# OATML-Markslab/ProteinGym

Measured on AMD Instinct MI355X. Metric: mutants scored/sec (ESM-1v 650M masked-marginal), higher is better.
Workload: dtype f16x3 (fp32 operands split into 2 fp16 planes, 3 fp16 MFMAs per product, fp32 accumulate)

## Files before the change

### proteingym_amd/csrc/api_esm.hip

```cpp
#include "model.h"

namespace pgmi {

int create_esm(pgmi_model* m, const pgmi_config* cfg, const float* w, int64_t n_weights) {
    const size_t D = cfg->embed_dim, F = cfg->ffn_dim, V = cfg->vocab, dh = m->dh, Da = m->Da;
    BlobCursor c(m, w, n_weights);
    c.upload(&m->embed_tokens, V * D);
    if (cfg->arch == PGMI_ARCH_ESM1B) c.upload(&m->embed_positions, (size_t)(cfg->max_positions + 2) * D);
    if (cfg->emb_layer_norm_before) {
        c.upload(&m->lnb_w, D);
        c.upload(&m->lnb_b, D);
    }
    auto slot = [&](size_t col) -> size_t { return rotate_half_slot(col, dh); };
    const float qscale = 1.0f / sqrtf((float)dh);
    m->layers.resize(cfg->layers);
    std::vector<float> wq(3 * Da * D, 0.0f), bq(3 * Da, 0.0f), wo_r(D * Da, 0.0f);
    for (int l = 0; l < cfg->layers; ++l) {
        Layer& L = m->layers[l];
        c.upload(&L.ln1_w, D);
        c.upload(&L.ln1_b, D);
        pack_qkv_slots(c.take(3 * (D * D + D)), D, Da, slot, qscale, wq.data(), bq.data());
        c.linear(&L.wqkv, &L.wqkv16, wq.data(), wq.size(), D);
        c.upload(&L.bqkv, bq.data(), bq.size());
        pack_out_cols(c.take(D * D), D, Da, slot, wo_r.data());
        c.linear(&L.wo, &L.wo16, wo_r.data(), wo_r.size(), Da);
        c.upload(&L.bo, D);
        c.upload(&L.ln2_w, D);
        c.upload(&L.ln2_b, D);
        c.linear(&L.w1, &L.w116, F * D, D);
        c.upload(&L.b1, F);
        c.linear(&L.w2, &L.w216, D * F, F);
        c.upload(&L.b2, D);
    }
    c.upload(&m->lna_w, D);
    c.upload(&m->lna_b, D);
    c.linear(&m->hd_w, &m->hd16, D * D, D);
    c.upload(&m->hd_b, D);
    c.upload(&m->hln_w, D);
    c.upload(&m->hln_b, D);
    c.upload(&m->head_b, V);
    m->head_w = m->embed_tokens;
    return c.finish();
}

int ensure_rotary(pgmi_model* m, int T) {
    if ((!esm2_rotary(m->cfg.arch) && m->cfg.arch != PGMI_ARCH_ESMC) || T <= m->rot_len) return PGMI_OK;
    return upload_rotate_half(m, std::max(T, 1026));
}

int upload_rotate_half(pgmi_model* m, int n) {
    const int rh = m->rot_halves;
    float inv[64];
    const int half = m->dh / 2;
    for (int i = 0; i < half; ++i) inv[i] = 1.0f / powf(10000.0f, (float)(2 * i) / (float)m->dh);
    return upload_rotary(m, n, rh, [&](int t, int g, int i) {
        const int j = (rh == 1) ? i : 32 * g + i;
        return j < half ? (float)t * inv[j] : 0.0f;
    });
}

int run_encoder(pgmi_model* m, int B, int T, const int32_t* keep, int n_keep, bool* compacted) {
    const pgmi_config& c = m->cfg;
    const int M = B * T, D = c.embed_dim, F = c.ffn_dim, N1 = m->fc1_cols, H = c.heads, Da = m->Da;
    hipStream_t s = m->stream;
    if (c.arch == PGMI_ARCH_ESM1B && T > c.max_positions) {
        set_error("Sequence length %d above maximum sequence length of %d", T, c.max_positions);
        return PGMI_EINVAL;
    }
    int rc = ensure_rotary(m, T);
    if (!rc) rc = reset_pad_keys(m, B, T);
    if (rc) return rc;
    {
        ProfScope p(m, PGMI_K_EMBED, 0, (double)M * D * 4);
        launch_seq_stats(m->tokens, B, T, m->embed_gather ? 0 : c.token_dropout, m->denom, m->pos_idx, m->kv_len, s, m->mask_id);
        if (m->embed_gather) launch_gather_rows(m->embed_tokens, m->tokens, M, D, m->x, s);
        else launch_embed(m->tokens, m->denom, m->pos_idx, m->embed_tokens, m->embed_positions, c.token_dropout, M, T, D, m->x, s, m->mask_id);
        if (m->lnb_w) {
            launch_layernorm(m->x, m->lnb_w, m->lnb_b, M, D, 1e-5f, m->x, s);
            launch_zero_pad_rows(m->tokens, M, D, m->x, s);
        }
    }
    const double ln_bytes = 2.0 * M * D * 4;
    const int prec = c.precision;
    const int mode16 = (prec == PGMI_PREC_F16X3) ? 1 : 2;
    for (int l = 0; l < c.layers; ++l) {
        const Layer& L = m->layers[l];
        { ProfScope p(m, PGMI_K_LAYERNORM, 0, ln_bytes);
          if (prec == PGMI_PREC_FP32) launch_layernorm(m->x, L.ln1_w, L.ln1_b, M, D, 1e-5f, m->h, s);
          else launch_layernorm16(m->x, L.ln1_w, L.ln1_b, M, D, 1e-5f, m->h16, m->h16_plane, mode16, s); }
        const bool fused_qkv = prec != PGMI_PREC_FP32 && !L.q_ln;
        { ProfScope p(m, PGMI_K_GEMM_QKV, 2.0 * M * 3 * D * D, 0);
          if (fused_qkv)
              rc = launch_gemm16_qkv(m->h16, m->h16_plane, L.wqkv16.p, L.wqkv16.plane, L.bqkv, M, Da, D, L.wqkv16.out_scale,
                                     m->qk16, m->qk16_plane, m->vt16, m->vt16_plane, m->rot_cos, m->rot_sin,
                                     esm2_rotary(c.arch), T, m->Hs, m->gemm_variant, s, m->rot_halves, prec == PGMI_PREC_BF16);
          else
              rc = linear(m, m->h, m->h16, m->h16_plane, L.wqkv, L.wqkv16, L.bqkv, nullptr, m->qkv, nullptr, 0, M, 3 * Da, D, EPI_NONE);
          if (rc) return rc; }
        { ProfScope p(m, PGMI_K_ATTENTION, 4.0 * M * T * D, L.q_ln ? (double)M * D * 20 : 0);
          if (L.q_ln && (rc = launch_qkln_prep(m->qkv, L.q_ln, L.k_ln, 1e-5f, m->rot_cos, m->rot_sin, B, T, H, m->qk16, m->qk16_plane,
                                               m->vt16, m->vt16_plane, s)))
              return rc;
          const bool v2 = prec != PGMI_PREC_FP32;
          if (esm2_rotary(c.arch) && !v2) launch_rotary(m->qkv, m->rot_cos, m->rot_sin, M, T, m->Hs, s, m->rot_halves);
          if (v2) {
              AttLaunch a;
              a.qk16 = m->qk16, a.qk_plane = m->qk16_plane, a.vt16 = m->vt16, a.vt_plane = m->vt16_plane;
              a.B = B, a.T = T, a.H = H, a.head_dim = m->rot_halves * kHeadDim;
              a.kv_len = m->kv_len;
              a.out = prec == PGMI_PREC_F16X3 ? ATT_OUT_SPLIT : ATT_OUT_BF16;
              a.ctx16 = m->h16;
              a.stream = s;
              rc = launch_attention_f16x3_v2(a);
          } else {
              rc = launch_attention_f32(m->qkv, m->kv_len, B, T, H, m->h, s, m->rot_halves * kHeadDim);
          }
          if (rc) return rc; }
        if (keep && m->keep_rows && l == c.layers - 1) {
            const int R = n_keep;
            ProfScope p(m, PGMI_K_KEPT_ROWS, 2.0 * R * D * (Da + N1 + F), 0);
            launch_gather_rows(m->x, keep, R, D, m->qkv, s);
            if (prec == PGMI_PREC_FP32) launch_gather_rows(m->h, keep, R, Da, m->g, s);
            else
                launch_gather_rows(reinterpret_cast<const float*>(m->h16), keep, R, prec == PGMI_PREC_F16X3 ? Da : Da / 2,
                                   reinterpret_cast<float*>(m->g16), s);
            rc = linear(m, m->g, m->g16, m->g16_plane, L.wo, L.wo16, L.bo, m->qkv, m->x, nullptr, 0, R, D, Da, EPI_NONE);
            if (rc) return rc;
            if (prec == PGMI_PREC_FP32) launch_layernorm(m->x, L.ln2_w, L.ln2_b, R, D, 1e-5f, m->h, s);
            else launch_layernorm16(m->x, L.ln2_w, L.ln2_b, R, D, 1e-5f, m->h16, m->h16_plane, mode16, s);
            rc = linear(m, m->h, m->h16, m->h16_plane, L.w1, L.w116, L.b1, nullptr,
                        prec == PGMI_PREC_FP32 ? m->g : nullptr, prec == PGMI_PREC_FP32 ? nullptr : m->g16, m->g16_plane,
                        R, N1, D, m->fc1_epi);
            if (rc) return rc;
            rc = linear(m, m->g, m->g16, m->g16_plane, L.w2, L.w216, L.b2, m->x, m->x, nullptr, 0, R, D, F, EPI_NONE);
            if (rc) return rc;
            if (compacted) *compacted = true;
            break;
        }
        { ProfScope p(m, PGMI_K_GEMM_OUT, 2.0 * M * D * D, 0);
          rc = linear(m, m->h, m->h16, m->h16_plane, L.wo, L.wo16, L.bo, m->x, m->x, nullptr, 0, M, D, Da, EPI_NONE);
          if (rc) return rc; }
        { ProfScope p(m, PGMI_K_LAYERNORM, 0, ln_bytes);
          if (prec == PGMI_PREC_FP32) launch_layernorm(m->x, L.ln2_w, L.ln2_b, M, D, 1e-5f, m->h, s);
          else launch_layernorm16(m->x, L.ln2_w, L.ln2_b, M, D, 1e-5f, m->h16, m->h16_plane, mode16, s); }
        { ProfScope p(m, PGMI_K_GEMM_FC1, 2.0 * M * N1 * D, 0);
          rc = linear(m, m->h, m->h16, m->h16_plane, L.w1, L.w116, L.b1, nullptr,
                      prec == PGMI_PREC_FP32 ? m->g : nullptr, prec == PGMI_PREC_FP32 ? nullptr : m->g16, m->g16_plane,
                      M, N1, D, m->fc1_epi);
          if (rc) return rc; }
        { ProfScope p(m, PGMI_K_GEMM_FC2, 2.0 * M * F * D, 0);
          rc = linear(m, m->g, m->g16, m->g16_plane, L.w2, L.w216, L.b2, m->x, m->x, nullptr, 0, M, D, F, EPI_NONE);
          if (rc) return rc; }
    }
    PGMI_HIP(hipGetLastError());
    return PGMI_OK;
}

int run_head(pgmi_model* m, int R, const int32_t* row_idx) {
    const pgmi_config& c = m->cfg;
    ProfScope p(m, PGMI_K_HEAD, 2.0 * R * c.embed_dim * (c.embed_dim + c.vocab), 0);
    int rc = head_hidden(m, R, row_idx);
    if (rc) return rc;
    launch_vocab_logsoftmax(m->g, m->head_w, m->head_b, R, c.embed_dim, c.vocab, m->lp, m->nonfinite, m->stream);
    PGMI_HIP(hipGetLastError());
    return PGMI_OK;
}

int head_hidden(pgmi_model* m, int R, const int32_t* row_idx) {
    const pgmi_config& c = m->cfg;
    const int D = c.embed_dim;
    hipStream_t s = m->stream;
    const int prec = c.precision;
    const float* src = m->x;
    if (row_idx) {
        launch_gather_rows(m->x, row_idx, R, D, m->h, s);
        src = m->h;
    }
    if (prec == PGMI_PREC_FP32) launch_layernorm(src, m->lna_w, m->lna_b, R, D, 1e-5f, m->h, s);
    else launch_layernorm16(src, m->lna_w, m->lna_b, R, D, 1e-5f, m->h16, m->h16_plane, prec == PGMI_PREC_F16X3 ? 1 : 2, s);
    int rc = linear(m, m->h, m->h16, m->h16_plane, m->hd_w, m->hd16, m->hd_b, nullptr, m->g, nullptr, 0, R, D, D, EPI_GELU);
    if (rc) return rc;
    launch_layernorm(m->g, m->hln_w, m->hln_b, R, D, 1e-5f, m->g, s);
    return PGMI_OK;
}


int run_rows(pgmi_model* m, int B, int T, int R, const int32_t* row_idx) {
    bool compacted = false;
    int rc = run_encoder(m, B, T, row_idx, R, &compacted);
    if (rc) return rc;
    return run_head(m, R, compacted ? nullptr : row_idx);
}

}

extern "C" {

int pgmi_token_logprobs(pgmi_model* m, const int32_t* tokens, int B, int T, float* out) {
    if (!m || !tokens || !out || B <= 0 || T <= 0) { set_error("bad argument"); return PGMI_EINVAL; }
    if (m->cfg.arch == PGMI_ARCH_SAPROT) { set_error("SaProt models are scored with pgmi_saprot_token_logprobs / pgmi_saprot_group_logprobs"); return PGMI_EINVAL; }
    if (T + 31 > m->max_rows) { set_error("T=%d exceeds workspace rows %d", T, m->max_rows); return PGMI_EINVAL; }
    int rc = check_tokens(tokens, B, T);
    if (rc) return rc;
    PGMI_HIP(hipSetDevice(m->device));
    const int V = m->cfg.vocab;
    rc = for_each_chunk(m, B, T, [&](int b0, int bc) {
        PGMI_HIP(hipMemcpyAsync(m->tokens, tokens + (size_t)b0 * T, (size_t)bc * T * 4, hipMemcpyHostToDevice, m->stream));
        int rc = run_rows(m, bc, T, bc * T, nullptr);
        if (rc) return rc;
        PGMI_HIP(hipMemcpyAsync(out + (size_t)b0 * T * V, m->lp, (size_t)bc * T * V * 4, hipMemcpyDeviceToHost, m->stream));
        return PGMI_OK;
    });
    return rc ? rc : check_nonfinite(m);
}

int pgmi_masked_logprobs(pgmi_model* m, const int32_t* tokens, const int32_t* mask_pos, int B, int T, float* out) {
    if (!m || !tokens || !mask_pos || !out || B <= 0 || T <= 0) { set_error("bad argument"); return PGMI_EINVAL; }
    if (m->cfg.arch == PGMI_ARCH_SAPROT) { set_error("SaProt models are scored with pgmi_saprot_token_logprobs / pgmi_saprot_group_logprobs"); return PGMI_EINVAL; }
    if (m->cfg.arch == PGMI_ARCH_ESMC && T + 31 > m->max_rows) { set_error("T=%d exceeds workspace rows %d", T, m->max_rows); return PGMI_EINVAL; }
    if (T > m->max_rows) { set_error("T=%d exceeds workspace rows %d", T, m->max_rows); return PGMI_EINVAL; }
    int rc = check_tokens(tokens, B, T);
    if (rc) return rc;
    for (int b = 0; b < B; ++b)
        if (mask_pos[b] < 0 || mask_pos[b] >= T) { set_error("mask_pos[%d]=%d out of range", b, mask_pos[b]); return PGMI_EINVAL; }
    PGMI_HIP(hipSetDevice(m->device));
    const int V = m->cfg.vocab;
    std::vector<int32_t> ridx;
    rc = for_each_chunk(m, B, T, [&](int b0, int bc) {
        ridx.resize(bc);
        for (int b = 0; b < bc; ++b) ridx[b] = b * T + mask_pos[b0 + b];
        PGMI_HIP(hipMemcpyAsync(m->tokens, tokens + (size_t)b0 * T, (size_t)bc * T * 4, hipMemcpyHostToDevice, m->stream));
        PGMI_HIP(hipMemcpyAsync(m->aux_i, mask_pos + b0, (size_t)bc * 4, hipMemcpyHostToDevice, m->stream));
        PGMI_HIP(hipMemcpyAsync(m->row_idx, ridx.data(), (size_t)bc * 4, hipMemcpyHostToDevice, m->stream));
        launch_apply_mask(m->tokens, m->aux_i, bc, T, m->stream);
        int rc = run_rows(m, bc, T, bc, m->row_idx);
        if (rc) return rc;
        PGMI_HIP(hipMemcpyAsync(out + (size_t)b0 * V, m->lp, (size_t)bc * V * 4, hipMemcpyDeviceToHost, m->stream));
        return PGMI_OK;
    });
    return rc ? rc : check_nonfinite(m);
}

int pgmi_assay_create(pgmi_model* m, const int32_t* wt_tokens, int n_tok, const int32_t* positions, int P,
                      int window, const int32_t* sub_pos, const int32_t* sub_wt, const int32_t* sub_mt,
                      const int64_t* mut_off, int64_t n_mut, pgmi_assay** out) {
    if (!out) { set_error("null out"); return PGMI_EINVAL; }
    *out = nullptr;
    if (!m || !wt_tokens || n_tok <= 0 || P < 0 || (P > 0 && !positions) || window <= 0 || n_mut < 0) { set_error("bad argument"); return PGMI_EINVAL; }
    if (m->cfg.arch == PGMI_ARCH_ESMC) { set_error("ESM C assays run through pgmi_masked_logprobs (their window rule is not pgmi_optimal_window)"); return PGMI_EINVAL; }
    if (m->cfg.arch == PGMI_ARCH_SAPROT) { set_error("SaProt assays run through pgmi_saprot_group_logprobs (position sets, no window)"); return PGMI_EINVAL; }
    for (int i = 0; i < n_tok; ++i)
        if (wt_tokens[i] < 0 || wt_tokens[i] >= PGMI_VOCAB || wt_tokens[i] == PGMI_TOK_PAD) { set_error("wt token %d invalid at %d", wt_tokens[i], i); return PGMI_EINVAL; }
    const int T = std::min(n_tok, window);
    if (T > m->max_rows) { set_error("T=%d exceeds workspace rows %d", T, m->max_rows); return PGMI_EINVAL; }
    std::vector<int32_t> ws(P), mr(P);
    for (int i = 0; i < P; ++i) {
        if (positions[i] < 0 || positions[i] >= n_tok) { set_error("position %d out of range", positions[i]); return PGMI_EINVAL; }
        int s, e;
        pgmi_optimal_window(positions[i], n_tok, window, &s, &e);
        if (e - s != T) { set_error("internal: window length %d != %d", e - s, T); return PGMI_EINVAL; }
        ws[i] = s;
        mr[i] = positions[i] - s;
    }
    const int64_t n_sub = n_mut ? mut_off[n_mut] : 0;
    for (int64_t k = 0; k < n_sub; ++k)
        if (sub_pos[k] < 0 || sub_pos[k] >= n_tok || sub_wt[k] < 0 || sub_wt[k] >= PGMI_VOCAB || sub_mt[k] < 0 || sub_mt[k] >= PGMI_VOCAB) {
            set_error("substitution %lld out of range", (long long)k);
            return PGMI_EINVAL;
        }
    PGMI_HIP(hipSetDevice(m->device));
    pgmi_assay* a = new pgmi_assay();
    a->m = m; a->n_tok = n_tok; a->P = P; a->T = T; a->n_mut = n_mut; a->n_sub = n_sub;
    int rc = dev_upload(a->allocs, &a->wt, wt_tokens, (size_t)n_tok);
    if (!rc) rc = dev_upload(a->allocs, &a->positions, positions, (size_t)P);
    if (!rc) rc = dev_upload(a->allocs, &a->win_start, ws.data(), (size_t)P);
    if (!rc) rc = dev_upload(a->allocs, &a->mask_rel, mr.data(), (size_t)P);
    if (!rc) rc = dev_upload(a->allocs, &a->sub_pos, sub_pos, (size_t)n_sub);
    if (!rc) rc = dev_upload(a->allocs, &a->sub_wt, sub_wt, (size_t)n_sub);
    if (!rc) rc = dev_upload(a->allocs, &a->sub_mt, sub_mt, (size_t)n_sub);
    if (!rc) rc = dev_upload(a->allocs, &a->mut_off, mut_off, (size_t)(n_mut + 1));
    if (!rc) rc = dev_alloc(a->allocs, &a->table, (size_t)n_tok * PGMI_VOCAB);
    if (!rc) rc = dev_alloc(a->allocs, &a->scores, (size_t)n_mut);
    if (rc) { pgmi_assay_destroy(a); return rc; }
    m->assays.push_back(a);
    *out = a;
    return PGMI_OK;
}

void pgmi_assay_destroy(pgmi_assay* a) {
    if (!a) return;
    if (a->m) {
        hipSetDevice(a->m->device);
        hipStreamSynchronize(a->m->stream);
        auto& v = a->m->assays;
        v.erase(std::remove(v.begin(), v.end(), a), v.end());
    }
    for (void* p : a->allocs) hipFree(p);
    delete a;
}

int pgmi_assay_run(pgmi_model* m, pgmi_assay* a, double* scores_host, float* table_host, double* scores_dev) {
    if (!m || !a || a->m != m) { set_error("bad model/assay handle (assay belongs to another or a destroyed model)"); return PGMI_EINVAL; }
    PGMI_HIP(hipSetDevice(m->device));
    hipStream_t s = m->stream;
    const int T = a->T, V = m->cfg.vocab;
    const int per = rows_per_chunk(m, T);
    launch_fill_f32(a->table, (int64_t)a->n_tok * V, NAN, s);
    for (int p0 = 0; p0 < a->P; p0 += per) {
        const int bc = std::min(per, a->P - p0);
        launch_make_masked_windows(a->wt, a->win_start + p0, a->mask_rel + p0, bc, T, m->tokens, s);
        launch_row_index(a->mask_rel + p0, bc, T, m->row_idx, s);
        int rc = run_rows(m, bc, T, bc, m->row_idx);
        if (rc) return rc;
        launch_scatter_rows(m->lp, a->positions + p0, bc, V, a->table, s);
    }
    {
        ProfScope p(m, PGMI_K_SCORE, 0, (double)a->n_sub * 20);
        launch_score_mutants(a->table, V, a->sub_pos, a->sub_wt, a->sub_mt, a->mut_off, a->n_mut, a->scores, s);
    }
    PGMI_HIP(hipGetLastError());
    if (scores_dev && a->n_mut) PGMI_HIP(hipMemcpyAsync(scores_dev, a->scores, (size_t)a->n_mut * 8, hipMemcpyDeviceToDevice, s));
    if (scores_host && a->n_mut) PGMI_HIP(hipMemcpyAsync(scores_host, a->scores, (size_t)a->n_mut * 8, hipMemcpyDeviceToHost, s));
    if (table_host) PGMI_HIP(hipMemcpyAsync(table_host, a->table, (size_t)a->n_tok * V * 4, hipMemcpyDeviceToHost, s));
    PGMI_HIP(hipStreamSynchronize(s));
    return check_nonfinite(m);
}

int pgmi_pppl_create(pgmi_model* m, const uint8_t* tokens, const int64_t* seq_off, int64_t n_seq, pgmi_pppl** out) {
    if (!out) { set_error("null out"); return PGMI_EINVAL; }
    *out = nullptr;
    if (!m || !tokens || !seq_off || n_seq <= 0 || n_seq > 0x7fffffff) { set_error("bad argument"); return PGMI_EINVAL; }
    if (m->cfg.arch != PGMI_ARCH_ESM1B && m->cfg.arch != PGMI_ARCH_ESM2) { set_error("pseudo-ppl needs an ESM-1b/1v/ESM2 model"); return PGMI_EINVAL; }
    if (seq_off[0] != 0) { set_error("seq_off[0] must be 0"); return PGMI_EINVAL; }
    for (int64_t n = 0; n < n_seq; ++n) {
        const int64_t len = seq_off[n + 1] - seq_off[n];
        if (len < 2 || len > (1 << 24)) { set_error("sequence %lld has %lld tokens", (long long)n, (long long)len); return PGMI_EINVAL; }
        const uint8_t* t = tokens + seq_off[n];
        for (int64_t i = 0; i < len; ++i)
            if (t[i] >= PGMI_VOCAB || t[i] == PGMI_TOK_PAD) { set_error("token id %d invalid at sequence %lld, position %lld", (int)t[i], (long long)n, (long long)i); return PGMI_EINVAL; }
    }
    PGMI_HIP(hipSetDevice(m->device));
    pgmi_pppl* q = new pgmi_pppl();
    q->m = m;
    q->N = n_seq;
    q->off.assign(seq_off, seq_off + n_seq + 1);
    int rc = dev_upload(q->allocs, &q->tok8, tokens, (size_t)seq_off[n_seq]);
    if (!rc) rc = dev_upload(q->allocs, &q->off_dev, seq_off, (size_t)n_seq + 1);
    if (rc) { for (void* p : q->allocs) hipFree(p); delete q; return rc; }
    m->pppls.push_back(q);
    *out = q;
    return PGMI_OK;
}

void pgmi_pppl_destroy(pgmi_pppl* q) {
    if (!q) return;
    if (q->m) {
        hipSetDevice(q->m->device);
        hipStreamSynchronize(q->m->stream);
        auto& v = q->m->pppls;
        v.erase(std::remove(v.begin(), v.end(), q), v.end());
    }
    for (void* p : q->allocs) hipFree(p);
    delete q;
}

int64_t pgmi_pppl_rows(const pgmi_pppl* q, int64_t first, int64_t count) {
    if (!q || first < 0 || count < 0 || first + count > q->N) return -1;
    int64_t r = 0;
    for (int64_t n = first; n < first + count; ++n) r += std::max<int64_t>(0, q->off[n + 1] - q->off[n] - 4);
    return r;
}

int pgmi_pppl_run(pgmi_model* m, pgmi_pppl* q, int64_t first, int64_t count, double* scores_host, float* terms_host,
                  double* scores_dev) {
    if (!m || !q || q->m != m) { set_error("bad model/library handle (library belongs to another or a destroyed model)"); return PGMI_EINVAL; }
    if (first < 0 || count <= 0 || first + count > q->N) { set_error("sequence range [%lld, %lld) outside the library of %lld", (long long)first, (long long)(first + count), (long long)q->N); return PGMI_EINVAL; }
    PGMI_HIP(hipSetDevice(m->device));
    hipStream_t s = m->stream;
    const int J = (int)count, V = m->cfg.vocab;
    std::vector<int32_t> sid(J);
    for (int j = 0; j < J; ++j) sid[j] = (int32_t)(first + j);
    auto len_of = [&](int32_t n) { return q->off[n + 1] - q->off[n]; };
    std::stable_sort(sid.begin(), sid.end(), [&](int32_t a, int32_t b) { return len_of(a) > len_of(b); });
    std::vector<int64_t> rp((size_t)J + 1);
    rp[0] = 0;
    for (int j = 0; j < J; ++j) rp[j + 1] = rp[j] + std::max<int64_t>(0, len_of(sid[j]) - 4);
    const int64_t R = rp[J];
    const int64_t Tmax = len_of(sid[0]);
    if (R > 0 && Tmax + 31 > m->max_rows) { set_error("T=%lld exceeds workspace rows %d", (long long)Tmax, m->max_rows); return PGMI_EINVAL; }
    if (R > 0 && m->cfg.arch == PGMI_ARCH_ESM1B && Tmax > m->cfg.max_positions) {
        set_error("Sequence length %lld above maximum sequence length of %d", (long long)Tmax, m->cfg.max_positions);
        return PGMI_EINVAL;
    }
    std::vector<void*> pool;
    auto cleanup = [&]() { for (void* p : pool) hipFree(p); };
    int32_t* d_sid = nullptr;
    int64_t* d_rp = nullptr;
    float* d_terms = nullptr;
    double* d_out = nullptr;
    int rc = dev_upload(pool, &d_sid, sid.data(), (size_t)J);
    if (!rc) rc = dev_upload(pool, &d_rp, rp.data(), (size_t)J + 1);
    if (!rc) rc = dev_alloc(pool, &d_terms, (size_t)R);
    if (!rc) rc = dev_alloc(pool, &d_out, (size_t)J);
    if (rc) { cleanup(); return rc; }
    q->last_rows = R; q->last_chunks = 0; q->last_tokens = 0; q->last_padded = 0;
    int j0 = 0;
    for (int64_t g0 = 0; g0 < R;) {
        while (rp[j0 + 1] <= g0) ++j0;
        const int T = (int)len_of(sid[j0]);
        const int bc = (int)std::min<int64_t>(rows_per_chunk(m, T), R - g0);
        launch_make_pppl_rows(q->tok8, q->off_dev, d_sid, d_rp, J, g0, bc, T, m->tokens, m->row_idx, m->aux_i, s);
        rc = run_rows(m, bc, T, bc, m->row_idx);
        if (rc) { hipStreamSynchronize(s); cleanup(); return rc; }
        launch_pppl_pick(m->lp, m->aux_i, bc, V, d_terms + g0, s);
        q->last_chunks += 1;
        q->last_padded += (int64_t)bc * T;
        g0 += bc;
        if ((q->last_chunks & 63) == 0 && g0 < R && (rc = check_nonfinite(m)) != PGMI_OK) { cleanup(); return rc; }
    }
    for (int j = 0; j < J; ++j) q->last_tokens += (rp[j + 1] - rp[j]) * len_of(sid[j]);
    {
        ProfScope p(m, PGMI_K_SCORE, 0, (double)R * 4);
        launch_pppl_sum(d_terms, d_rp, d_sid, J, first, d_out, s);
    }
    hipError_t e = hipGetLastError();
    if (e == hipSuccess && scores_dev) e = hipMemcpyAsync(scores_dev, d_out, (size_t)J * 8, hipMemcpyDeviceToDevice, s);
    if (e == hipSuccess && scores_host) e = hipMemcpyAsync(scores_host, d_out, (size_t)J * 8, hipMemcpyDeviceToHost, s);
    std::vector<float> sorted_terms;
    if (e == hipSuccess && terms_host && R > 0) {
        sorted_terms.resize((size_t)R);
        e = hipMemcpyAsync(sorted_terms.data(), d_terms, (size_t)R * 4, hipMemcpyDeviceToHost, s);
    }
    if (e == hipSuccess) e = hipStreamSynchronize(s);
    cleanup();
    if (e != hipSuccess) { set_error("pseudo-ppl run failed: %s", hipGetErrorString(e)); return PGMI_EHIP; }
    if (terms_host && R > 0) {
        std::vector<int64_t> dst((size_t)J + 1, 0);
        for (int k = 0; k < J; ++k) dst[k + 1] = dst[k] + std::max<int64_t>(0, len_of((int32_t)(first + k)) - 4);
        for (int j = 0; j < J; ++j)
            std::copy(sorted_terms.begin() + rp[j], sorted_terms.begin() + rp[j + 1], terms_host + dst[sid[j] - first]);
    }
    return check_nonfinite(m);
}

int pgmi_pppl_stats(const pgmi_pppl* q, int64_t* rows, int64_t* chunks, int64_t* tokens, int64_t* padded_tokens) {
    if (!q) { set_error("null library"); return PGMI_EINVAL; }
    if (rows) *rows = q->last_rows;
    if (chunks) *chunks = q->last_chunks;
    if (tokens) *tokens = q->last_tokens;
    if (padded_tokens) *padded_tokens = q->last_padded;
    return PGMI_OK;
}

}
```

### proteingym_amd/csrc/api_model.hip

```cpp
#include "model.h"

namespace pgmi {

static thread_local char g_err[1024] = "";
void set_error(const char* fmt, ...) {
    va_list ap;
    va_start(ap, fmt);
    vsnprintf(g_err, sizeof(g_err), fmt, ap);
    va_end(ap);
}

int prof_drain(pgmi_model* m) {
    if (m->events_used == 0) return PGMI_OK;
    PGMI_HIP(hipStreamSynchronize(m->stream));
    for (size_t i = 0; i < m->events_used; ++i) {
        float ms = 0.f;
        PGMI_HIP(hipEventElapsedTime(&ms, m->events[i].start, m->events[i].stop));
        m->prof_ms[m->events[i].cls] += ms;
    }
    m->events_used = 0;
    return PGMI_OK;
}

int check_cfg(const pgmi_config* c) {
    if (!c) { set_error("null config"); return PGMI_EINVAL; }
    if (c->abi_version != PGMI_ABI_VERSION) { set_error("ABI version mismatch: got %d, library is %d", c->abi_version, PGMI_ABI_VERSION); return PGMI_EINVAL; }
    if (c->arch != PGMI_ARCH_ESM1B && c->arch != PGMI_ARCH_ESM2 && c->arch != PGMI_ARCH_TRANCEPTION && c->arch != PGMI_ARCH_MSA &&
        c->arch != PGMI_ARCH_PROGEN2 && c->arch != PGMI_ARCH_GPT && c->arch != PGMI_ARCH_ESMC && c->arch != PGMI_ARCH_SAPROT) { set_error("unknown arch %d", c->arch); return PGMI_EINVAL; }
    if (c->layers <= 0 || c->embed_dim <= 0 || c->heads <= 0 || c->ffn_dim <= 0) { set_error("non-positive model dimension"); return PGMI_EINVAL; }
    if (c->arch == PGMI_ARCH_ESMC) {
        if (c->precision != PGMI_PREC_F16X3) { set_error("ESM C is available in precision f16x3 only"); return PGMI_EINVAL; }
        if (c->embed_dim % 32 || c->embed_dim != c->heads * kHeadDim) { set_error("ESM C needs head_dim 64 and d %% 32 == 0 (embed_dim %d, heads %d)", c->embed_dim, c->heads); return PGMI_EINVAL; }
        if (c->embed_dim > 2048) { set_error("ESM C: embed_dim %d above the 2048 this build supports", c->embed_dim); return PGMI_EINVAL; }
        if (c->ffn_dim % 32) { set_error("ESM C: the SwiGLU hidden width %d must be a multiple of 32", c->ffn_dim); return PGMI_EINVAL; }
        if (c->vocab != PGMI_ESMC_VOCAB) { set_error("ESM C vocab must be %d", PGMI_ESMC_VOCAB); return PGMI_EINVAL; }
        return PGMI_OK;
    }
    {
        const int dh = c->embed_dim / c->heads;
        const bool pg2 = c->arch == PGMI_ARCH_PROGEN2;
        const bool esm_layout = c->arch == PGMI_ARCH_ESM1B || c->arch == PGMI_ARCH_ESM2 || c->arch == PGMI_ARCH_GPT || c->arch == PGMI_ARCH_SAPROT;
        const bool ok = c->embed_dim % c->heads == 0 &&
                        (dh == kHeadDim || (dh < kHeadDim && dh % 2 == 0 && esm_layout) || (dh == 2 * kHeadDim && esm_layout) ||
                         (pg2 && dh % 2 == 0 && dh <= 4 * kHeadDim));
        if (pg2 && !ok && c->embed_dim % c->heads == 0 && dh > 4 * kHeadDim) {
            set_error("unsupported head_dim %d (embed_dim %d / heads %d): ProGen2 runs even head dims up to 256", dh, c->embed_dim, c->heads);
            return PGMI_EINVAL;
        }
        if (!ok) { set_error("unsupported head_dim %d (embed_dim %d / heads %d): this build supports head_dim 64, even head dims below 64 and head_dim 128 (ESM)", dh, c->embed_dim, c->heads); return PGMI_EINVAL; }
    }
    if (c->embed_dim % 32 || c->ffn_dim % 32) { set_error("embed_dim and ffn_dim must be multiples of 32"); return PGMI_EINVAL; }
    if (c->arch == PGMI_ARCH_TRANCEPTION) {
        if (c->vocab != 25) { set_error("Tranception vocab must be 25"); return PGMI_EINVAL; }
        if (c->heads % 4) { set_error("Invalid number of heads. Tranception requires the number of heads to be a multiple of 4."); return PGMI_EINVAL; }
        if (c->precision != PGMI_PREC_F16X3) { set_error("Tranception is available in precision f16x3 only"); return PGMI_EINVAL; }
        if (c->max_positions <= 0) { set_error("Tranception needs max_positions = n_ctx"); return PGMI_EINVAL; }
    } else if (c->arch == PGMI_ARCH_PROGEN2) {
        if (c->vocab != PGMI_PG2_VOCAB) { set_error("ProGen2 vocab must be %d", PGMI_PG2_VOCAB); return PGMI_EINVAL; }
        if (c->heads % 8) { set_error("ProGen2 needs the number of heads to be a multiple of 8 (mp_num = 8), got %d", c->heads); return PGMI_EINVAL; }
        if (c->precision != PGMI_PREC_F16X3) { set_error("ProGen2 is available in precision f16x3 only"); return PGMI_EINVAL; }
        if (c->max_positions <= 0) { set_error("ProGen2 needs max_positions = n_positions"); return PGMI_EINVAL; }
    } else if (c->arch == PGMI_ARCH_GPT) {
        if (c->vocab < 2) { set_error("causal decoder vocab must be at least 2, got %d", c->vocab); return PGMI_EINVAL; }
        if (c->precision != PGMI_PREC_F16X3) { set_error("the causal decoder (RITA / ProtGPT2) is available in precision f16x3 only"); return PGMI_EINVAL; }
        if (c->max_positions <= 0) { set_error("the causal decoder needs max_positions = n_positions / max_seq_len"); return PGMI_EINVAL; }
    } else if (c->arch == PGMI_ARCH_SAPROT) {
        if (c->vocab != PGMI_SAPROT_VOCAB) { set_error("SaProt vocab must be %d (5 specials + 21 x 21 residue tokens)", PGMI_SAPROT_VOCAB); return PGMI_EINVAL; }
        if (c->max_positions != 0) { set_error("SaProt has rotary positions: max_positions must be 0"); return PGMI_EINVAL; }
    } else if (c->vocab != PGMI_VOCAB) { set_error("vocab must be %d", PGMI_VOCAB); return PGMI_EINVAL; }
    if (c->arch == PGMI_ARCH_ESM1B && c->max_positions <= 0) { set_error("ESM-1b arch needs max_positions"); return PGMI_EINVAL; }
    if (c->arch == PGMI_ARCH_MSA) {
        if (c->max_positions <= 0) { set_error("MSA Transformer needs max_positions"); return PGMI_EINVAL; }
        if (c->embed_dim != c->heads * kHeadDim) { set_error("MSA Transformer: head_dim must be 64"); return PGMI_EINVAL; }
        if (c->precision != PGMI_PREC_F16X3) { set_error("MSA Transformer is available in precision f16x3 only"); return PGMI_EINVAL; }
    }
    if (c->precision != PGMI_PREC_FP32 && c->precision != PGMI_PREC_F16X3 && c->precision != PGMI_PREC_BF16) { set_error("unknown precision %d", c->precision); return PGMI_EINVAL; }
    if (c->precision == PGMI_PREC_BF16 && (c->embed_dim % 64 || c->ffn_dim % 64)) { set_error("precision bf16 needs embed_dim and ffn_dim to be multiples of 64"); return PGMI_EINVAL; }
    return PGMI_OK;
}

int check_tokens(const int32_t* tokens, int B, int T, int n_ids) {
    for (int b = 0; b < B; ++b) {
        const int32_t* t = tokens + (size_t)b * T;
        bool seen_pad = false;
        if (t[0] == PGMI_TOK_PAD) { set_error("sequence %d is empty (all <pad>)", b); return PGMI_EINVAL; }
        for (int i = 0; i < T; ++i) {
            if (t[i] < 0 || t[i] >= n_ids) { set_error("token id %d out of range at [%d,%d]", t[i], b, i); return PGMI_EINVAL; }
            if (t[i] == PGMI_TOK_PAD) seen_pad = true;
            else if (seen_pad) { set_error("interior <pad> at [%d,%d]: only trailing padding is supported", b, i); return PGMI_EINVAL; }
        }
    }
    return PGMI_OK;
}

int check_vocab(const int32_t* tokens, int B, int T, int V) {
    for (int b = 0; b < B; ++b)
        for (int t = 0; t < T; ++t) {
            const int tk = tokens[(size_t)b * T + t];
            if (tk < 0 || tk >= V) { set_error("token id %d out of range at [%d,%d]", tk, b, t); return PGMI_EINVAL; }
        }
    return PGMI_OK;
}

int env_int(const char* name, int dflt) {
    const char* v = getenv(name);
    return v ? atoi(v) : dflt;
}

int make_w16(std::vector<void*>& pool, const float* host, size_t n, size_t K, int precision, hipStream_t s, W16* out) {
    float mx = 0.f;
    for (size_t i = 0; i < n; ++i) mx = std::max(mx, fabsf(host[i]));
    float scale = 1.0f;
    const int planes = (precision == PGMI_PREC_F16X3) ? 2 : 1;
    if (precision == PGMI_PREC_F16X3 && mx > 0.f && std::isfinite(mx)) scale = exp2f(floorf(log2f(16384.0f / mx)));
    float* tmp = nullptr;
    hipError_t e = hipMalloc(reinterpret_cast<void**>(&tmp), n * sizeof(float));
    if (e != hipSuccess) { set_error("hipMalloc failed: %s", hipGetErrorString(e)); return PGMI_ENOMEM; }
    int rc = dev_alloc(pool, &out->p, n * planes);
    if (rc) { hipFree(tmp); return rc; }
    e = hipMemcpy(tmp, host, n * sizeof(float), hipMemcpyHostToDevice);
    if (e == hipSuccess) {
        launch_split16(tmp, (int64_t)n, scale, precision == PGMI_PREC_BF16 ? 1 : 0, (int)K, out->p, s);
        e = hipStreamSynchronize(s);
    }
    hipFree(tmp);
    if (e != hipSuccess) { set_error("weight split failed: %s", hipGetErrorString(e)); return PGMI_EHIP; }
    out->plane = n;
    out->out_scale = 1.0f / scale;
    return PGMI_OK;
}

int linear(pgmi_model* m, const float* in32, const unsigned short* in16, size_t in_plane, const float* W32,
           const W16& w16, const float* bias, const float* residual, float* out32, unsigned short* out16,
           size_t out_plane, int M, int N, int K, int epi) {
    if (m->cfg.precision == PGMI_PREC_FP32)
        return launch_gemm_f32(in32, W32, bias, residual, out32, M, N, K, epi, m->stream);
    const bool bf = m->cfg.precision == PGMI_PREC_BF16;
    return launch_gemm16(in16, in_plane, w16.p, w16.plane, bias, residual, out32, out16, out_plane, M, N, K, epi,
                         w16.out_scale, bf ? 1 : 2, bf, m->gemm_variant, m->stream);
}

int check_nonfinite(pgmi_model* m) {
    if (m->cfg.precision == PGMI_PREC_FP32) return PGMI_OK;
    int32_t flag = 0;
    PGMI_HIP(hipMemcpyAsync(&flag, m->nonfinite, 4, hipMemcpyDeviceToHost, m->stream));
    PGMI_HIP(hipStreamSynchronize(m->stream));
    if (flag) {
        PGMI_HIP(hipMemsetAsync(m->nonfinite, 0, 4, m->stream));
        set_error("non-finite log-probabilities: an activation left the fp16/bf16 range in precision mode %d; "
                  "re-run with precision fp32", m->cfg.precision);
        return PGMI_EOVERFLOW;
    }
    return PGMI_OK;
}

int reset_pad_keys(pgmi_model* m, int B, int T) {
    if (!m->vt16 || (B == m->last_B && T == m->last_T)) return PGMI_OK;
    PGMI_HIP(hipMemsetAsync(m->vt16, 0, m->vt16_plane * 2 * sizeof(unsigned short), m->stream));
    m->last_B = B;
    m->last_T = T;
    return PGMI_OK;
}

}

extern "C" {

int pgmi_abi_version(void) { return PGMI_ABI_VERSION; }

const char* pgmi_last_error(void) { return g_err; }

int pgmi_device_count(void) {
    int n = 0;
    if (hipGetDeviceCount(&n) != hipSuccess) return 0;
    return n;
}

int64_t pgmi_weight_count(const pgmi_config* c) {
    if (!c || c->layers <= 0 || c->embed_dim <= 0 || c->ffn_dim <= 0) return -1;
    const int64_t D = c->embed_dim, F = c->ffn_dim, V = c->vocab;
    if (c->arch == PGMI_ARCH_TRANCEPTION) {
        const int64_t conv = 3 * ((64 * 3 + 64) + (64 * 5 + 64) + (64 * 7 + 64));
        return V * D + (int64_t)c->layers * (2 * D + (D * 3 * D + 3 * D) + conv + (D * D + D) + 2 * D + (D * F + F) + (F * D + D)) + 2 * D + V * D;
    }
    if (c->arch == PGMI_ARCH_PROGEN2)
        return V * D + (int64_t)c->layers * (2 * D + 3 * D * D + D * D + (F * D + F) + (D * F + D)) + 2 * D + V * D + V;
    if (c->arch == PGMI_ARCH_GPT) return -1;
    if (c->arch == PGMI_ARCH_ESMC) return esmc_weight_count(c);
    if (c->arch == PGMI_ARCH_MSA) {
        const int64_t attn = 2 * D + 4 * (D * D + D);
        return V * D + (int64_t)(c->max_positions + 2) * D + 1024 * D + 2 * D +
               (int64_t)c->layers * (2 * attn + 2 * D + (F * D + F) + (D * F + D)) + 2 * D + (D * D + D) + 2 * D + V;
    }
    int64_t n = V * D;
    if (c->arch == PGMI_ARCH_ESM1B) n += (int64_t)(c->max_positions + 2) * D;
    if (c->emb_layer_norm_before) n += 2 * D;
    n += (int64_t)c->layers * (2 * D + 4 * (D * D + D) + 2 * D + (F * D + F) + (D * F + D));
    n += 2 * D + (D * D + D) + 2 * D + V;
    return n;
}

int pgmi_model_create(const pgmi_config* cfg, const float* w, int64_t n_weights, int device, pgmi_model** out) {
    if (cfg && cfg->arch == PGMI_ARCH_PROGEN2) {
        if (out) *out = nullptr;
        set_error("ProGen2 models are created with pgmi_pg2_model_create (it takes rotary_dim)");
        return PGMI_EINVAL;
    }
    if (cfg && cfg->arch == PGMI_ARCH_GPT) {
        if (out) *out = nullptr;
        set_error("causal decoder models are created with pgmi_gpt_model_create (it takes pos_kind)");
        return PGMI_EINVAL;
    }
    if (cfg && cfg->arch == PGMI_ARCH_SAPROT) {
        if (out) *out = nullptr;
        set_error("SaProt models are created with pgmi_saprot_model_create (it takes the tokenizer's <mask> id)");
        return PGMI_EINVAL;
    }
    return model_create(cfg, w, n_weights, device, out, 0);
}

}

namespace pgmi {

static int alloc_workspace(pgmi_model* m) {
    const pgmi_config& c = m->cfg;
    const size_t R = m->max_rows, D = c.embed_dim, F = c.ffn_dim, V = c.vocab, Da = m->Da;
    const size_t Dw = std::max(D, Da);
    const bool f32mode = c.precision == PGMI_PREC_FP32;
    int rc = PGMI_OK;
    auto alloc = [&](auto** p, size_t n) { if (!rc) rc = dev_alloc(m->allocs, p, n); };
    alloc(&m->x, R * D);
    alloc(&m->h, R * Dw);
    alloc(&m->qkv, R * 3 * Da);
    alloc(&m->g, R * (f32mode ? std::max(F, D) : D));
    if (!f32mode) {
        const size_t planes = c.precision == PGMI_PREC_F16X3 ? 2 : 1;
        m->h16_plane = R * Dw;
        m->g16_plane = R * F;
        alloc(&m->h16, m->h16_plane * planes);
        alloc(&m->g16, m->g16_plane * planes);
    }
    alloc(&m->nonfinite, (size_t)1);
    if (!f32mode) {
        m->qk16_plane = R * 2 * Da;
        m->vt16_plane = R * Da;
        alloc(&m->qk16, m->qk16_plane * 2);
        alloc(&m->vt16, m->vt16_plane * 2);
    }
    if (c.arch == PGMI_ARCH_MSA) {
        alloc(&m->xt, R * D);
        alloc(&m->msa_kv_len, (size_t)2048);
    }
    alloc(&m->lp, (c.arch == PGMI_ARCH_GPT && V > kWave ? (size_t)m->gpt_head_rows : R) * V);
    alloc(&m->denom, R);
    alloc(&m->tokens, R);
    alloc(&m->pos_idx, R);
    alloc(&m->kv_len, R);
    alloc(&m->row_idx, R);
    alloc(&m->aux_i, R);
    if (rc) return rc;
    PGMI_HIP(hipMemset(m->nonfinite, 0, 4));
    if (m->vt16) PGMI_HIP(hipMemset(m->vt16, 0, m->vt16_plane * 2 * sizeof(unsigned short)));
    return PGMI_OK;
}

int model_create(const pgmi_config* cfg, const float* w, int64_t n_weights, int device, pgmi_model** out, int arch_arg) {
    if (!out) { set_error("null out"); return PGMI_EINVAL; }
    *out = nullptr;
    int rc = check_cfg(cfg);
    if (rc) return rc;
    const int64_t need = cfg->arch == PGMI_ARCH_GPT ? gpt_weight_count(cfg, arch_arg) : pgmi_weight_count(cfg);
    if (need < 0) { set_error("causal decoder pos_kind %d: must be PGMI_GPT_POS_ROTARY or PGMI_GPT_POS_LEARNED", arch_arg); return PGMI_EINVAL; }
    if (!w || n_weights != need) {
        set_error("weight blob has %lld elements, config needs %lld", (long long)n_weights, (long long)need);
        return PGMI_EINVAL;
    }
    const int ndev = pgmi_device_count();
    if (ndev <= 0) { set_error("no HIP device visible (libpgmi has no CPU fallback)"); return PGMI_ENODEV; }
    if (device < 0 || device >= ndev) { set_error("device %d out of range (%d visible)", device, ndev); return PGMI_EINVAL; }
    PGMI_HIP(hipSetDevice(device));
    pgmi_model* m = new pgmi_model();
    m->cfg = *cfg;
    m->device = device;
    if (hipStreamCreateWithFlags(&m->stream, hipStreamNonBlocking) != hipSuccess) { set_error("hipStreamCreate failed"); delete m; return PGMI_EHIP; }
    m->dh = cfg->embed_dim / cfg->heads;
    m->rot_halves = m->dh > 2 * kHeadDim ? 4 : m->dh > kHeadDim ? 2 : 1;
    m->Hs = cfg->heads * m->rot_halves;
    m->Da = m->Hs * kHeadDim;
    m->ln_eps = cfg->ln_eps > 0.f ? cfg->ln_eps : 1e-5f;
    m->max_rows = std::max(cfg->max_rows > 0 ? cfg->max_rows : 98304, 2048);
    const size_t V = cfg->vocab;
    const std::vector<float> zeros(std::max({3 * (size_t)m->Da, (V + 63) / 64 * 64, (size_t)cfg->embed_dim, V, (size_t)cfg->heads}), 0.0f);
    rc = dev_upload(m->allocs, &m->zeros, zeros.data(), zeros.size());
    m->fc1_cols = cfg->ffn_dim;
    if (!rc) switch (cfg->arch) {
        case PGMI_ARCH_TRANCEPTION: rc = create_tranception(m, cfg, w, n_weights); break;
        case PGMI_ARCH_MSA: rc = create_msa(m, cfg, w, n_weights); break;
        case PGMI_ARCH_PROGEN2: rc = create_progen2(m, cfg, w, n_weights, arch_arg); break;
        case PGMI_ARCH_GPT: rc = create_gpt(m, cfg, w, n_weights, arch_arg); break;
        case PGMI_ARCH_ESMC: rc = create_esmc(m, cfg, w, n_weights); break;
        case PGMI_ARCH_SAPROT: rc = create_saprot(m, cfg, w, n_weights, arch_arg); break;
        default: rc = create_esm(m, cfg, w, n_weights);
    }
    if (!rc) rc = alloc_workspace(m);
    if (rc) { pgmi_model_destroy(m); return rc; }
    m->keep_rows = env_int("PGMI_KEEP_ROWS", 1);
    gemm_options_from_env();
    m->gemm_variant = env_int("PGMI_GEMM_VARIANT", 0);
    *out = m;
    return PGMI_OK;
}

}

extern "C" {

void pgmi_model_destroy(pgmi_model* m) {
    if (!m) return;
    hipSetDevice(m->device);
    if (m->stream) hipStreamSynchronize(m->stream);
    for (pgmi_assay* a : m->assays) {
        for (void* p : a->allocs) hipFree(p);
        a->allocs.clear();
        a->m = nullptr;
    }
    m->assays.clear();
    for (pgmi_pppl* q : m->pppls) {
        for (void* p : q->allocs) hipFree(p);
        q->allocs.clear();
        q->m = nullptr;
    }
    m->pppls.clear();
    for (auto& e : m->events) { hipEventDestroy(e.start); hipEventDestroy(e.stop); }
    for (void* p : m->allocs) hipFree(p);
    if (m->stream) hipStreamDestroy(m->stream);
    delete m;
}

int pgmi_model_device(const pgmi_model* m) { return m ? m->device : -1; }

int pgmi_set_option(const char* name, int64_t value) {
    if (!name) { set_error("null option name"); return PGMI_EINVAL; }
    int rc = gemm_set_option(name, (long long)value);
    if (rc) rc = att_set_option(name, (long long)value);
    if (rc) rc = eve_set_option(name, (long long)value);
    if (rc) set_error("unknown option '%s' (gemm_half_tail, gemm_max_rows, att_xcd_local, att_v3, eve_max_rows, eve_fixed_sample)", name);
    return rc;
}

int pgmi_synchronize(pgmi_model* m) {
    if (!m) { set_error("null model"); return PGMI_EINVAL; }
    PGMI_HIP(hipStreamSynchronize(m->stream));
    return PGMI_OK;
}

int pgmi_profile_enable(pgmi_model* m, int on) {
    if (!m) { set_error("null model"); return PGMI_EINVAL; }
    int rc = prof_drain(m);
    m->prof = on != 0;
    return rc;
}

int pgmi_profile_reset(pgmi_model* m) {
    if (!m) { set_error("null model"); return PGMI_EINVAL; }
    int rc = prof_drain(m);
    for (int i = 0; i < PGMI_K_COUNT; ++i) { m->prof_ms[i] = 0; m->prof_n[i] = 0; m->prof_flops[i] = 0; m->prof_bytes[i] = 0; }
    return rc;
}

int pgmi_profile_get(pgmi_model* m, int k, double* ms, int64_t* launches, double* flops, double* bytes) {
    if (!m || k < 0 || k >= PGMI_K_COUNT) { set_error("bad argument"); return PGMI_EINVAL; }
    int rc = prof_drain(m);
    if (rc) return rc;
    if (ms) *ms = m->prof_ms[k];
    if (launches) *launches = m->prof_n[k];
    if (flops) *flops = m->prof_flops[k];
    if (bytes) *bytes = m->prof_bytes[k];
    return PGMI_OK;
}

}
```

### proteingym_amd/csrc/attention_f16.hip

```cpp
#include <stdlib.h>
#include <string.h>
#include <algorithm>

#include "attention_f16_common.h"

namespace pgmi {

template <int WPB, int OUT, int NSTG, int DH = 64, bool RAG = false, int DO = DH>
__global__ __launch_bounds__(WPB * 64) void attention_f16x3_v2_kernel(
    const unsigned short* __restrict__ qk16, size_t qk_plane, const unsigned short* __restrict__ vt16,
    size_t vt_plane, const int32_t* __restrict__ kv_len, const float* __restrict__ slopes, int T, int H,
    int Tp, float* __restrict__ ctx, unsigned short* __restrict__ ctx16, RagMap rag, int dense_nblk, int nseq) {
    constexpr float defer_thr = kAttDefer;
    constexpr int NT = WPB * 64;
    constexpr int KCPR = DH / 8;
    constexpr int KCH = AKT * KCPR, VCH = DO * 4;
    constexpr int NSL = DH / DO;
    static_assert(NSL == 1 || (OUT == ATT_OUT_SPLIT && !RAG), "sliced context: split-plane output of dense launches only");
    constexpr int STG_CH = 2 * KCH + 2 * VCH;
    constexpr int NWI = STG_CH / 64;
    static_assert(NWI % WPB == 0, "the wave-instructions of a stage divide evenly over the waves");
    constexpr int NDMA = NWI / WPB;
    constexpr int NS = DH / 16, ND = DO / 32;
    extern __shared__ __attribute__((aligned(16))) u32x4 lds[];

    int b, h, qblk_dense, hs;
    if (RAG) {
        b = rag.ent_seq[blockIdx.x];
        hs = blockIdx.y;
        qblk_dense = 0;
    } else if (dense_nblk > 0) {
        const int pair = xcd_local_pair(dense_nblk, qblk_dense);
        if (pair >= nseq * H * NSL) return;
        b = pair / (H * NSL);
        hs = pair - b * (H * NSL);
    } else {
        b = blockIdx.z;
        hs = blockIdx.y;
        qblk_dense = blockIdx.x;
    }
    h = hs / NSL;
    const int d0 = (hs - h * NSL) * DO;
    const int tid = threadIdx.x, lane = tid & 63;
    const int wave = __builtin_amdgcn_readfirstlane(tid >> 6);
    const int r = lane & 31, kh = lane >> 5;
    const int D = H * DH;
    const int Tk = (!RAG && kv_len) ? kv_len[b] : T;
    const int p0 = RAG ? rag.seq_p[b] : 0, a0 = p0 & ~(AKT - 1), kt0 = a0 / AKT;
    const int qblk = RAG ? rag.ent_j[blockIdx.x] : qblk_dense;
    const int row0 = RAG ? rag.seq_q[b] : b * T, rrow0 = RAG ? rag.seq_q[rag.seq_root[b]] : 0;
    const int orow0 = RAG ? rag.seq_off[b] - p0 : b * T;
    const int Tpo = RAG ? (T - a0 + 31) / 32 * 32 : Tp;
    const int q0 = a0 + (qblk * WPB + wave) * 32;
    const bool active = q0 < T;

    constexpr bool q_lds = NSTG >= 3;
    u32x4 qh[NS], ql[NS];
    if (!q_lds) {
        const int qrow = min(q0 + r, T - 1);
        const unsigned short* qp = qk16 + ((size_t)row0 + (qrow - a0)) * (2 * D) + h * DH + kh * 8;
#pragma unroll
        for (int s = 0; s < NS; ++s) {
            qh[s] = *reinterpret_cast<const u32x4*>(qp + s * 16);
            ql[s] = *reinterpret_cast<const u32x4*>(qp + qk_plane + s * 16);
        }
    }

    const size_t seq_halfs = (size_t)T * (2 * D), vt_halfs = (size_t)DH * Tp;
    const unsigned long long qk_bytes = std::min<unsigned long long>(0xFFFFFFFFull, (unsigned long long)qk_plane * 2ull + seq_halfs * 2ull);
    const unsigned long long vt_bytes = std::min<unsigned long long>(0xFFFFFFFFull, (unsigned long long)vt_plane * 2ull + vt_halfs * 2ull);
    const __amdgpu_buffer_rsrc_t rsQK = operand_rsrc(qk16 + (size_t)row0 * (2 * D), qk_bytes);
    const __amdgpu_buffer_rsrc_t rsVT = operand_rsrc(vt16 + (RAG ? (size_t)rag.seq_vt[b] + (size_t)h * DH * Tpo : ((size_t)b * H + h) * vt_halfs), vt_bytes);
    const __amdgpu_buffer_rsrc_t rsQKr = operand_rsrc(qk16 + (size_t)rrow0 * (2 * D), qk_bytes);
    const __amdgpu_buffer_rsrc_t rsVTr = operand_rsrc(vt16 + (RAG ? (size_t)rag.seq_vt[rag.seq_root[b]] + (size_t)h * DH * Tp : (size_t)0), vt_bytes);
    const bool causal = slopes != nullptr;
    const int last_q = min(T, a0 + (qblk * WPB + WPB) * 32);
    const int nkt = causal ? (min(Tk, last_q) + AKT - 1) / AKT : (Tk + AKT - 1) / AKT;
    int voff[NDMA], voff_last[NDMA], voff_root[NDMA], sbase[NDMA], sstep[NDMA], slot0[NDMA];
    bool is_k[NDMA];
#pragma unroll
    for (int i = 0; i < NDMA; ++i) {
        int wi = wave + WPB * i;
        if (wi >= NWI) wi -= NWI;
        slot0[i] = wi * 64;
        is_k[i] = wi < 2 * KCH / 64;
        if (is_k[i]) {
            const int p = wi / (KCH / 64), key = ((wi % (KCH / 64)) * 64 + lane) / KCPR;
            const int c = (lane % KCPR) ^ k_swizzle<DH>(key);
            voff[i] = voff_root[i] = key * (2 * D) * 2 + c * 16;
            voff_last[i] = min(key, T - 1 - (nkt - 1) * AKT) * (2 * D) * 2 + c * 16;
            sbase[i] = (int)((unsigned int)p * (unsigned int)qk_plane * 2u + (unsigned int)(D + h * DH) * 2u);
            sstep[i] = AKT * (2 * D) * 2;
        } else {
            const int wv = wi - 2 * KCH / 64, p = wv / (VCH / 64), g = (wv % (VCH / 64)) * 64 + lane;
            const int d = g >> 2, c = (g & 3) ^ ((d >> 2) & 3);
            voff[i] = voff_last[i] = (d0 + d) * Tpo * 2 + c * 16;
            voff_root[i] = (d0 + d) * Tp * 2 + c * 16;
            sbase[i] = (int)((unsigned int)p * (unsigned int)vt_plane * 2u);
            sstep[i] = (AKT / 8) * 16;
        }
    }
    auto issue_tile = [&](int kt, int buf) {
        u32x4* base = lds + buf * STG_CH;
        const bool from_root = RAG && kt < kt0;
#pragma unroll
        for (int i = 0; i < NDMA; ++i) {
            const int vo = from_root ? voff_root[i] : ((kt == nkt - 1) ? voff_last[i] : voff[i]);
            const int so = sbase[i] + (from_root ? kt : kt - kt0) * sstep[i];
            if (is_k[i]) __builtin_amdgcn_raw_ptr_buffer_load_lds(from_root ? rsQKr : rsQK, (__attribute__((address_space(3))) void*)(base + slot0[i]), 16, vo, so, 0, 0);
            else __builtin_amdgcn_raw_ptr_buffer_load_lds(from_root ? rsVTr : rsVT, (__attribute__((address_space(3))) void*)(base + slot0[i]), 16, vo, so, 0, 0);
        }
    };

    constexpr float kLog2e = 1.4426950408889634f;
    const float slope2 = causal ? slopes[h] * kLog2e : 0.0f;
    if (q_lds) {
        issue_tile(0, 0);
        u32x4* qbase = lds + STG_CH + wave * (2 * KCH);
        if (active) {
            constexpr int NQ = 2 * KCH / 64;
#pragma unroll
            for (int i = 0; i < NQ; ++i) {
                const int f = i * 64 + lane, pq = f / KCH, row = (f % KCH) / KCPR;
                const int c = (f % KCPR) ^ k_swizzle<DH>(row);
                const int vo = (int)(((unsigned int)(min(q0 + row, T - 1) - a0) * (unsigned int)(2 * D) + (unsigned int)(h * DH)) * 2u + (unsigned int)c * 16u);
                const int so = (int)((unsigned int)pq * (unsigned int)qk_plane * 2u);
                __builtin_amdgcn_raw_ptr_buffer_load_lds(rsQK, (__attribute__((address_space(3))) void*)(qbase + i * 64), 16, vo, so, 0, 0);
            }
        }
        asm volatile("s_waitcnt vmcnt(0)" ::: "memory");
        if (active) {
#pragma unroll
            for (int s = 0; s < NS; ++s) {
                const int ci = r * KCPR + ((2 * s + kh) ^ k_swizzle<DH>(r));
                qh[s] = qbase[ci];
                ql[s] = qbase[KCH + ci];
            }
        }
        asm volatile("s_waitcnt lgkmcnt(0)" ::: "memory");
        __builtin_amdgcn_s_barrier();
        asm volatile("" ::: "memory");
#pragma unroll
        for (int t = 1; t < NSTG - 1; ++t)
            if (t < nkt) issue_tile(t, t);
    } else {
#pragma unroll
        for (int t = 0; t < NSTG - 1; ++t)
            if (t < nkt) issue_tile(t, t);
    }

    f32x16 om[ND], oc[ND];
#pragma unroll
    for (int dt = 0; dt < ND; ++dt)
#pragma unroll
        for (int v = 0; v < 16; ++v) { om[dt][v] = 0.f; oc[dt][v] = 0.f; }
    float m_run = -INFINITY, l_run = 0.f;
    constexpr float kInvLo = 1.0f / kLoScale;

    const f32x16 zero16 = {0.f, 0.f, 0.f, 0.f, 0.f, 0.f, 0.f, 0.f, 0.f, 0.f, 0.f, 0.f, 0.f, 0.f, 0.f, 0.f};
    auto wanted = [&](int kt) -> bool { return active && !(causal && kt * AKT > q0 + 31); };
    auto scores = [&](int buf, f32x16& sm, f32x16& sc) {
        const u32x4* Kb = lds + buf * STG_CH;
#pragma unroll
        for (int s = 0; s < NS; ++s) {
            const int ci = r * KCPR + ((2 * s + kh) ^ k_swizzle<DH>(r));
            const u32x4 kfh = Kb[ci], kfl = Kb[KCH + ci];
            sc = mfma_h(kfh, ql[s], s == 0 ? zero16 : sc);
            sc = mfma_h(kfl, qh[s], sc);
            sm = mfma_h(kfh, qh[s], s == 0 ? zero16 : sm);
        }
    };
    auto wait_tile = [&](int younger) {
        if (younger >= 2) asm volatile("s_waitcnt vmcnt(%0)" ::"n"(2 * NDMA) : "memory");
        else if (younger == 1) asm volatile("s_waitcnt vmcnt(%0)" ::"n"(NDMA) : "memory");
        else asm volatile("s_waitcnt vmcnt(0)" ::: "memory");
    };
    int cur = 0;
    for (int kt = 0; kt < nkt; ++kt) {
        wait_tile(min(NSTG - 2, nkt - 1 - kt));
        __builtin_amdgcn_s_barrier();
        asm volatile("" ::: "memory");
        if (kt + NSTG - 1 < nkt) issue_tile(kt + NSTG - 1, (cur == 0) ? NSTG - 1 : cur - 1);
        if (wanted(kt)) {
            const u32x4* Vb = lds + cur * STG_CH + 2 * KCH;
            f32x16 sm, sc;
            scores(cur, sm, sc);
            float st[16];
            if (causal) {
                const float kb = (float)(kt * AKT + 4 * kh);
#pragma unroll
                for (int v = 0; v < 16; ++v)
                    st[v] = fmaf(slope2, kb + (float)((v & 3) + 8 * (v >> 2)), fmaf(sc[v], kInvLo, sm[v]));
                if (kt * AKT + AKT - 1 > q0) {
#pragma unroll
                    for (int v = 0; v < 16; ++v) {
                        const int key = kt * AKT + (v & 3) + 8 * (v >> 2) + 4 * kh;
                        if (key > q0 + r) st[v] = -INFINITY;
                    }
                }
            } else {
#pragma unroll
                for (int v = 0; v < 16; ++v) st[v] = fmaf(sc[v], kInvLo, sm[v]);
            }
            if (kt * AKT + AKT > Tk) {
#pragma unroll
                for (int v = 0; v < 16; ++v) {
                    const int key = kt * AKT + (v & 3) + 8 * (v >> 2) + 4 * kh;
                    if (key >= Tk) st[v] = -INFINITY;
                }
            }
            float mloc = st[0];
#pragma unroll
            for (int v = 1; v < 16; ++v) mloc = fmaxf(mloc, st[v]);
            {
                const unsigned int mu = __builtin_bit_cast(unsigned int, mloc);
                const auto sw = __builtin_amdgcn_permlane32_swap(mu, mu, false, false);
                const unsigned int s0 = sw[0], s1 = sw[1];
                mloc = fmaxf(__builtin_bit_cast(float, s0), __builtin_bit_cast(float, s1));
            }
            const float m_new = fmaxf(m_run, mloc);
            if (!__all(m_new <= m_run + defer_thr)) {
                const bool moved = m_new > m_run + defer_thr;
                const float alpha = moved ? __builtin_amdgcn_exp2f(m_run - m_new) : 1.0f;
                l_run *= alpha;
#pragma unroll
                for (int dt = 0; dt < ND; ++dt)
#pragma unroll
                    for (int v = 0; v < 16; ++v) { om[dt][v] *= alpha; oc[dt][v] *= alpha; }
                if (moved) m_run = m_new;
            }
            const float mb = m_run - 10.0f;
            typedef float f32x2 __attribute__((ext_vector_type(2)));
#pragma unroll
            for (int v = 0; v < 16; v += 2) {
                const f32x2 dlt = f32x2{st[v], st[v + 1]} - f32x2{mb, mb};
                st[v] = __builtin_amdgcn_exp2f(dlt[0]);
                st[v + 1] = __builtin_amdgcn_exp2f(dlt[1]);
            }
            l_run += ((st[0] + st[1]) + (st[2] + st[3])) + ((st[4] + st[5]) + (st[6] + st[7])) +
                     (((st[8] + st[9]) + (st[10] + st[11])) + ((st[12] + st[13]) + (st[14] + st[15])));
#pragma unroll
            for (int m = 0; m < 2; ++m) {
                u32x4 ph, pl;
#pragma unroll
                for (int e = 0; e < 4; ++e) {
                    const u32x2 p = split_p(st[8 * m + 2 * e], st[8 * m + 2 * e + 1]);
                    ph[e] = p[0];
                    pl[e] = p[1];
                }
#pragma unroll
                for (int dt = 0; dt < ND; ++dt) {
                    const int ci = v_chunk(dt * 32 + r, m, kh);
                    const u32x4 vfh = Vb[ci], vfl = Vb[VCH + ci];
                    oc[dt] = mfma_h(vfh, pl, oc[dt]);
                    oc[dt] = mfma_h(vfl, ph, oc[dt]);
                    om[dt] = mfma_h(vfh, ph, om[dt]);
                }
            }
        }
        cur = (cur == NSTG - 1) ? 0 : cur + 1;
    }

    if (active) {
        const float l_tot = l_run + __shfl_xor(l_run, 32);
        const float inv = 1.0f / l_tot;
        const bool row_ok = q0 + r < T && q0 + r >= p0;
        const size_t orow = (size_t)(orow0 + max(min(q0 + r, T - 1), p0));
        if (OUT == ATT_OUT_BF16) store_ctx_bf16<ND>(om, oc, inv, kInvLo, row_ok, ctx16 + orow * (size_t)D + (size_t)h * DH, kh);
        else if (OUT == ATT_OUT_SPLIT) store_ctx_split<ND>(om, oc, inv, kInvLo, row_ok, ctx16 + orow * (size_t)(2 * D) + (size_t)((h * DH + d0) / 32) * 64, kh);
        else if (row_ok) store_ctx_f32<ND>(om, oc, inv, kInvLo, ctx + (size_t)(orow0 + q0 + r) * D + (size_t)h * DH + 4 * kh);
    }
}


using Att16v2Kernel = decltype(&attention_f16x3_v2_kernel<4, ATT_OUT_F32, 3, 64, false, 64>);
struct Att16v2Inst { int wpb, out, head_dim; bool rag; Att16v2Kernel fn; size_t lds_bytes; };
template <int WPB, int OUT, int NSTG, int DH, bool RAG = false, int DO = DH>
static constexpr Att16v2Inst att16v2_inst() {
    return {WPB, OUT, DH, RAG, attention_f16x3_v2_kernel<WPB, OUT, NSTG, DH, RAG, DO>, (size_t)NSTG * (8 * DH + 8 * DO) * 16};
}
static const Att16v2Inst kAtt16v2[] = {
    att16v2_inst<1, ATT_OUT_F32, 3, 64>(),   att16v2_inst<2, ATT_OUT_F32, 3, 64>(),   att16v2_inst<4, ATT_OUT_F32, 3, 64>(),
    att16v2_inst<1, ATT_OUT_SPLIT, 3, 64>(), att16v2_inst<2, ATT_OUT_SPLIT, 3, 64>(), att16v2_inst<4, ATT_OUT_SPLIT, 3, 64>(),
    att16v2_inst<1, ATT_OUT_BF16, 3, 64>(),  att16v2_inst<2, ATT_OUT_BF16, 3, 64>(),  att16v2_inst<4, ATT_OUT_BF16, 3, 64>(),
    att16v2_inst<1, ATT_OUT_SPLIT, 3, 64, true>(), att16v2_inst<2, ATT_OUT_SPLIT, 3, 64, true>(), att16v2_inst<4, ATT_OUT_SPLIT, 3, 64, true>(),
    att16v2_inst<4, ATT_OUT_F32, 3, 128>(),  att16v2_inst<4, ATT_OUT_SPLIT, 3, 128>(), att16v2_inst<4, ATT_OUT_BF16, 3, 128>(),
    att16v2_inst<4, ATT_OUT_SPLIT, 2, 256, false, 128>(),
};

static int launch_att16v2(const AttLaunch& a, int wpb, dim3 grid, const RagMap* rag, int dense_nblk) {
    for (const Att16v2Inst& k : kAtt16v2) {
        if (k.wpb != wpb || k.out != a.out || k.head_dim != a.head_dim || k.rag != (rag != nullptr)) continue;
        if (k.lds_bytes > 65536) {
            hipError_t e = hipFuncSetAttribute(reinterpret_cast<const void*>(k.fn), hipFuncAttributeMaxDynamicSharedMemorySize, (int)k.lds_bytes);
            if (e != hipSuccess) { set_error("hipFuncSetAttribute: %s", hipGetErrorString(e)); return PGMI_EHIP; }
        }
        hipLaunchKernelGGL(k.fn, grid, dim3(wpb * 64), k.lds_bytes, a.stream, a.qk16, a.qk_plane, a.vt16, a.vt_plane, a.kv_len, a.slopes,
                           a.T, a.H, (a.T + 31) / 32 * 32, a.ctx, a.ctx16, rag ? *rag : RagMap{}, dense_nblk, a.B);
        PGMI_HIP(hipGetLastError());
        return PGMI_OK;
    }
    set_error("attention_f16x3_v2: no kernel for %d waves, output %d, head_dim %d%s", wpb, (int)a.out, a.head_dim, rag ? ", ragged" : "");
    return PGMI_EINVAL;
}

static int g_att_xcd_local = -1;
int att_set_option(const char* name, long long value) {
    if (!strcmp(name, "att_xcd_local")) { g_att_xcd_local = (int)value; return PGMI_OK; }
    if (!strcmp(name, "att_v3")) { att_v3_set_option((int)value); return PGMI_OK; }
    return PGMI_EINVAL;
}
static dim3 dense_grid(int nblk, int H, int B, int* dense_nblk) {
    if (g_att_xcd_local == 0 || (g_att_xcd_local < 0 && nblk < 2)) { *dense_nblk = 0; return dim3(nblk, H, B); }
    *dense_nblk = nblk;
    const long long pairs = (long long)H * B, groups = (pairs + 7) / 8;
    return dim3((unsigned)(groups * 8 * nblk), 1, 1);
}

int att16_waves_per_block(int T) {
    const int n32 = (T + 31) / 32, nblk = (n32 + 3) / 4;
    const int wpb = (n32 + nblk - 1) / nblk;
    return wpb == 3 ? 4 : wpb;
}

static int check_operand_range(const char* who, const AttLaunch& a) {
    const unsigned long long Tp = (unsigned long long)(a.T + 31) / 32 * 32;
    const unsigned long long seq_bytes = (unsigned long long)a.T * 2ull * (unsigned long long)a.H * (unsigned long long)a.head_dim * 2ull;
    const unsigned long long vt_bytes = (unsigned long long)a.head_dim * Tp * 2ull;
    if ((unsigned long long)a.qk_plane * 2ull + seq_bytes >= (1ull << 32) || (unsigned long long)a.vt_plane * 2ull + vt_bytes >= (1ull << 32)) {
        set_error("%s: operand planes of %zu / %zu halfs exceed the 32-bit offset range of the K / V^T DMA "
                  "(plane stride + one sequence must stay below 4 GiB: create the model with a smaller max_rows)", who, a.qk_plane, a.vt_plane);
        return PGMI_EINVAL;
    }
    return PGMI_OK;
}

int launch_attention_f16x3_v2(const AttLaunch& a) {
    const int B = a.B, T = a.T, H = a.H, head_dim = a.head_dim;
    if (B <= 0 || T <= 0 || H <= 0 || a.out < ATT_OUT_F32 || a.out > ATT_OUT_BF16 || (head_dim != 64 && head_dim != 128 && head_dim != 256)) {
        set_error("attention_f16x3_v2: bad arguments B=%d T=%d H=%d out=%d head_dim=%d", B, T, H, (int)a.out, head_dim);
        return PGMI_EINVAL;
    }
    const int n32 = (T + 31) / 32, Tp = n32 * 32;
    int rc = check_operand_range("attention_f16x3_v2", a);
    if (rc) return rc;
    int dn = 0;
    if (head_dim == 256) {
        if (a.qkv || a.conv || !a.slopes || a.out != ATT_OUT_SPLIT) { set_error("attention_f16x3_v2: head_dim 256 is the causal, fused-QKV, split-plane-output flavour only"); return PGMI_EINVAL; }
        const dim3 grid = dense_grid((n32 + 3) / 4, 2 * H, B, &dn);
        return launch_att16v2(a, 4, grid, nullptr, dn);
    }
    if (head_dim == 128) {
        if (a.qkv || a.conv) { set_error("attention_f16x3_v2: head_dim 128 needs operands from the fused QKV projection"); return PGMI_EINVAL; }
        const dim3 grid = dense_grid((n32 + 3) / 4, H, B, &dn);
        return launch_att16v2(a, 4, grid, nullptr, dn);
    }
    if (a.qkv && a.conv && a.rotary) { set_error("attention_f16x3_v2: depth-wise convolution and rotary together are not a model this library knows"); return PGMI_EINVAL; }
    if (a.qkv && a.conv && H % 4) { set_error("attention_f16x3_v2: the depth-wise convolution has four head groups, H = %d is not a multiple of 4", H); return PGMI_EINVAL; }
    if (a.qkv && a.conv)
        launch_qkv_prep_conv(dim3(n32, H, B), a.stream, a.qkv, a.conv, T, H, Tp, a.qk16, a.qk_plane, a.vt16, a.vt_plane, nullptr);
    else if (a.qkv)
        launch_qkv_prep(dim3(n32, H, B), a.stream, a.qkv, a.cos_t, a.sin_t, a.rotary, T, H, Tp, a.qk16, a.qk_plane, a.vt16, a.vt_plane);
    const int wpb = att16_waves_per_block(T);
    const dim3 grid = dense_grid((n32 + wpb - 1) / wpb, H, B, &dn);
    return att_v3_serves(a) ? launch_att16v3(a, wpb, grid, dn) : launch_att16v2(a, wpb, grid, nullptr, dn);
}

int launch_attention_tr_ragged(const AttLaunch& a, const AttRagged& rg) {
    const int T = a.T, H = a.H;
    if (T <= 0 || H <= 0 || !a.qkv || !a.conv || !a.slopes || a.head_dim != 64 || a.out != ATT_OUT_SPLIT || rg.n_tiles <= 0 || rg.n_blocks <= 0) {
        set_error("attention_tr_ragged: bad arguments T=%d H=%d tiles=%d blocks=%d", T, H, rg.n_tiles, rg.n_blocks);
        return PGMI_EINVAL;
    }
    const int rc = check_operand_range("attention_tr_ragged", a);
    if (rc) return rc;
    const RagMap tiles{rg.seq_off, rg.seq_p, rg.seq_q, rg.seq_root, rg.seq_vt, rg.tile_seq, rg.tile_j};
    launch_qkv_prep_conv(dim3(rg.n_tiles, H, 1), a.stream, a.qkv, a.conv, T, H, (T + 31) / 32 * 32, a.qk16, a.qk_plane, a.vt16, a.vt_plane, &tiles);
    const RagMap rag{rg.seq_off, rg.seq_p, rg.seq_q, rg.seq_root, rg.seq_vt, rg.blk_seq, rg.blk_j};
    return launch_att16v2(a, att16_waves_per_block(T), dim3(rg.n_blocks, H, 1), &rag, 0);
}

}
```

### proteingym_amd/csrc/attention_f16_v3.hip

```cpp
#include <stdlib.h>
#include <string.h>
#include <algorithm>

#include "attention_f16_common.h"

namespace pgmi {

template <int WPB, int OUT>
__global__ __launch_bounds__(WPB * 64, 2) void attention_f16x3_v3_kernel(
    const unsigned short* __restrict__ qk16, size_t qk_plane, const unsigned short* __restrict__ vt16, size_t vt_plane,
    const int32_t* __restrict__ kv_len, int T, int H, int Tp, float* __restrict__ ctx, unsigned short* __restrict__ ctx16,
    int dense_nblk, int nseq) {
    constexpr float defer_thr = kAttDefer;
    constexpr int DH = 64, NSTG = 3, KCPR = 8, KCH = AKT * KCPR, VCH = DH * 4, STG_CH = 2 * KCH + 2 * VCH;
    constexpr int NWI = STG_CH / 64, NDMA = (NWI + WPB - 1) / WPB, NS = 4, ND = 2;
    extern __shared__ __attribute__((aligned(16))) u32x4 lds[];
    int b, h, qblk;
    if (dense_nblk > 0) {
        const int pair = xcd_local_pair(dense_nblk, qblk);
        if (pair >= nseq * H) return;
        b = pair / H;
        h = pair - b * H;
    } else {
        b = blockIdx.z;
        h = blockIdx.y;
        qblk = blockIdx.x;
    }
    const int tid = threadIdx.x, lane = tid & 63;
    const int wave = __builtin_amdgcn_readfirstlane(tid >> 6);
    const int r = lane & 31, kh = lane >> 5;
    const int D = H * DH;
    const int Tk = kv_len ? kv_len[b] : T;
    const int q0 = (qblk * WPB + wave) * 32;
    const bool active = q0 < T;
    const int nkt = (Tk + AKT - 1) / AKT;
    const size_t seq_halfs = (size_t)T * (2 * D), vt_halfs = (size_t)DH * Tp;
    const unsigned long long qk_bytes = std::min<unsigned long long>(0xFFFFFFFFull, (unsigned long long)qk_plane * 2ull + seq_halfs * 2ull);
    const unsigned long long vt_bytes = std::min<unsigned long long>(0xFFFFFFFFull, (unsigned long long)vt_plane * 2ull + vt_halfs * 2ull);
    const __amdgpu_buffer_rsrc_t rsQK = operand_rsrc(qk16 + (size_t)b * seq_halfs, qk_bytes);
    const __amdgpu_buffer_rsrc_t rsVT = operand_rsrc(vt16 + ((size_t)b * H + h) * vt_halfs, vt_bytes);

    static_assert(WPB == 1 || WPB == 2 || WPB == 4, "the DMA map needs WPB to divide 8");
    constexpr int NK = 8 / WPB;
    int kvoff[NK], krow[NK], vvoff[NDMA - NK];
#pragma unroll
    for (int i = 0; i < NK; ++i) {
        const int q4 = (wave + WPB * i) & 3;
        const int key = q4 * 8 + (lane >> 3);
        krow[i] = key;
        kvoff[i] = ((lane & 7) ^ k_swizzle<DH>(key)) * 16;
    }
#pragma unroll
    for (int i = 0; i < NDMA - NK; ++i) {
        const int q4 = (wave + WPB * (i + NK)) & 3;
        const int g = q4 * 64 + lane, d = g >> 2, c = (g & 3) ^ ((d >> 2) & 3);
        vvoff[i] = d * Tp * 2 + c * 16;
    }
    auto issue_piece = [&](int i, int m, int stage, bool on) {
        u32x4* base = lds + stage * STG_CH;
        const int kk = min(m, nkt - 1), vv = min(max(m - 2, 0), nkt - 1);
        if (i < NK) {
            const int wi = wave + WPB * i, p = (WPB * i) >> 2;
            const int kr = krow[i < NK ? i : 0], ko = kvoff[i < NK ? i : 0];
            const int vo = on ? min(kk * AKT + kr, T - 1) * (2 * D) * 2 + ko : -16;
            const int so = (int)((unsigned int)p * (unsigned int)qk_plane * 2u + (unsigned int)(D + h * DH) * 2u);
            __builtin_amdgcn_raw_ptr_buffer_load_lds(rsQK, (__attribute__((address_space(3))) void*)(base + wi * 64), 16, vo, so, 0, 0);
        } else {
            const int wi = wave + WPB * i, p = (WPB * i - 8) >> 2;
            const int so = (int)((unsigned int)p * (unsigned int)vt_plane * 2u) + vv * ((AKT / 8) * 16);
            const int vv0 = vvoff[i >= NK ? i - NK : 0];
            const int vo = on ? vv0 : -16;
            __builtin_amdgcn_raw_ptr_buffer_load_lds(rsVT, (__attribute__((address_space(3))) void*)(base + wi * 64), 16, vo, so, 0, 0);
        }
    };
    auto issue_bundle = [&](int m, int stage, bool on) {
#pragma unroll
        for (int i = 0; i < NDMA; ++i) issue_piece(i, m, stage, on);
    };
    const int last_bundle = nkt + 1;

    issue_bundle(0, 0, true);
    u32x4 qh[NS], ql[NS];
    {
        u32x4* qbase = lds + STG_CH + wave * (2 * KCH);
        if (active) {
            constexpr int NQ = 2 * KCH / 64;
#pragma unroll
            for (int i = 0; i < NQ; ++i) {
                const int f = i * 64 + lane, pq = f / KCH, row = (f % KCH) / KCPR;
                const int c = (f % KCPR) ^ k_swizzle<DH>(row);
                const int vo = (int)(((unsigned int)min(q0 + row, T - 1) * (unsigned int)(2 * D) + (unsigned int)(h * DH)) * 2u + (unsigned int)c * 16u);
                const int so = (int)((unsigned int)pq * (unsigned int)qk_plane * 2u);
                __builtin_amdgcn_raw_ptr_buffer_load_lds(rsQK, (__attribute__((address_space(3))) void*)(qbase + i * 64), 16, vo, so, 0, 0);
            }
        }
        asm volatile("s_waitcnt vmcnt(0)" ::: "memory");
        if (active) {
#pragma unroll
            for (int s = 0; s < NS; ++s) {
                const int ci = r * KCPR + ((2 * s + kh) ^ k_swizzle<DH>(r));
                qh[s] = qbase[ci];
                ql[s] = qbase[KCH + ci];
            }
        }
        asm volatile("s_waitcnt lgkmcnt(0)" ::: "memory");
        __builtin_amdgcn_s_barrier();
        asm volatile("" ::: "memory");
    }
    issue_bundle(1, 1, true);
    issue_bundle(2, 2, true);

    f32x16 om[ND], oc[ND], sm, sc;
#pragma unroll
    for (int dt = 0; dt < ND; ++dt)
#pragma unroll
        for (int v = 0; v < 16; ++v) { om[dt][v] = 0.f; oc[dt][v] = 0.f; }
#pragma unroll
    for (int v = 0; v < 16; ++v) { sm[v] = 0.f; sc[v] = 0.f; }
    u32x4 ph[2], pl[2];
#pragma unroll
    for (int m = 0; m < 2; ++m)
#pragma unroll
        for (int e = 0; e < 4; ++e) { ph[m][e] = 0u; pl[m][e] = 0u; }
    float m_run = -INFINITY, l_run = 0.f;
    constexpr float kInvLo = 1.0f / kLoScale;
    const f32x16 zero16 = {0.f, 0.f, 0.f, 0.f, 0.f, 0.f, 0.f, 0.f, 0.f, 0.f, 0.f, 0.f, 0.f, 0.f, 0.f, 0.f};
    typedef float f32x2 __attribute__((ext_vector_type(2)));
    typedef _Float16 h4 __attribute__((ext_vector_type(4)));

    auto vfrag = [&](const u32x4* Vb, int m, u32x4 (&fh)[ND], u32x4 (&fl)[ND]) {
#pragma unroll
        for (int dt = 0; dt < ND; ++dt) {
            const int ci = v_chunk(dt * 32 + r, m, kh);
            fh[dt] = Vb[ci];
            fl[dt] = Vb[VCH + ci];
        }
    };
    auto kfrag = [&](const u32x4* Kb, int s, u32x4& kh_, u32x4& kl_) {
        const int ci = r * KCPR + ((2 * s + kh) ^ k_swizzle<DH>(r));
        kh_ = Kb[ci];
        kl_ = Kb[KCH + ci];
    };
    auto pv = [&](int m, const u32x4 (&fh)[ND], const u32x4 (&fl)[ND]) {
#pragma unroll
        for (int dt = 0; dt < ND; ++dt) {
            oc[dt] = mfma_h(fh[dt], pl[m], oc[dt]);
            oc[dt] = mfma_h(fl[dt], ph[m], oc[dt]);
            om[dt] = mfma_h(fh[dt], ph[m], om[dt]);
        }
    };
    auto split_pm = [&](const float (&st)[16], int m, int e) {
        const u32x2 p = split_p(st[8 * m + 2 * e], st[8 * m + 2 * e + 1]);
        ph[m][e] = p[0];
        pl[m][e] = p[1];
    };
    bool pend = false;
    float pend_alpha = 1.0f;
    auto apply_pending = [&]() {
        if (pend) {
#pragma unroll
            for (int dt = 0; dt < ND; ++dt)
#pragma unroll
                for (int v = 0; v < 16; ++v) { om[dt][v] *= pend_alpha; oc[dt][v] *= pend_alpha; }
        }
    };
    auto step = [&](auto MKc, int kt, const u32x4* stage, int dma_stage) {
        constexpr bool MK = decltype(MKc)::value;
        apply_pending();
        const u32x4* Kb = stage;
        const u32x4* Vb = stage + 2 * KCH;
        u32x4 va_h[ND], va_l[ND], vb_h[ND], vb_l[ND];
        u32x4 k0h, k0l, k1h, k1l;
        float st[16];
#define PGMI_SLOT() __builtin_amdgcn_sched_barrier(0)
        vfrag(Vb, 0, va_h, va_l);
        vfrag(Vb, 1, vb_h, vb_l);
#pragma unroll
        for (int v = 0; v < 16; ++v) st[v] = fmaf(sc[v], kInvLo, sm[v]);
        if constexpr (MK) {
#pragma unroll
            for (int v = 0; v < 16; ++v) {
                const int key = kt * AKT + (v & 3) + 8 * (v >> 2) + 4 * kh;
                if (key >= Tk) st[v] = -INFINITY;
            }
        }
        float ma = st[0];
#pragma unroll
        for (int v = 1; v < 8; ++v) ma = fmaxf(ma, st[v]);
        PGMI_SLOT();
        oc[0] = mfma_h(va_h[0], pl[0], oc[0]);
        float mloc = st[8];
#pragma unroll
        for (int v = 9; v < 16; ++v) mloc = fmaxf(mloc, st[v]);
        mloc = fmaxf(mloc, ma);
        PGMI_SLOT();
        oc[0] = mfma_h(va_l[0], ph[0], oc[0]);
        {
            const unsigned int mu = __builtin_bit_cast(unsigned int, mloc);
            const auto sw = __builtin_amdgcn_permlane32_swap(mu, mu, false, false);
            const unsigned int s0 = sw[0], s1 = sw[1];
            mloc = fmaxf(__builtin_bit_cast(float, s0), __builtin_bit_cast(float, s1));
        }
        const float m_new = fmaxf(m_run, mloc);
        PGMI_SLOT();
        om[0] = mfma_h(va_h[0], ph[0], om[0]);
        const bool moved = m_new > m_run + defer_thr;
        pend = !__all(m_new <= m_run + defer_thr);
        pend_alpha = moved ? __builtin_amdgcn_exp2f(m_run - m_new) : 1.0f;
        l_run *= pend_alpha;
        asm volatile("" : "+v"(l_run));
        m_run = moved ? m_new : m_run;
        const float mb = m_run - 10.0f;
        PGMI_SLOT();
        auto exp_pairs = [&](int v0) {
#pragma unroll
            for (int v = v0; v < v0 + 4; v += 2) {
                const f32x2 dlt = f32x2{st[v], st[v + 1]} - f32x2{mb, mb};
                st[v] = __builtin_amdgcn_exp2f(dlt[0]);
                st[v + 1] = __builtin_amdgcn_exp2f(dlt[1]);
            }
        };
        oc[1] = mfma_h(va_h[1], pl[0], oc[1]);
        exp_pairs(0);
        PGMI_SLOT();
        oc[1] = mfma_h(va_l[1], ph[0], oc[1]);
        exp_pairs(4);
        PGMI_SLOT();
        om[1] = mfma_h(va_h[1], ph[0], om[1]);
        exp_pairs(8);
        PGMI_SLOT();
        oc[0] = mfma_h(vb_h[0], pl[1], oc[0]);
        exp_pairs(12);
        PGMI_SLOT();
        oc[0] = mfma_h(vb_l[0], ph[1], oc[0]);
        const float sa = ((st[0] + st[1]) + (st[2] + st[3])) + ((st[4] + st[5]) + (st[6] + st[7]));
        PGMI_SLOT();
        om[0] = mfma_h(vb_h[0], ph[1], om[0]);
        kfrag(Kb, 0, k0h, k0l);
        l_run += sa + (((st[8] + st[9]) + (st[10] + st[11])) + ((st[12] + st[13]) + (st[14] + st[15])));
        PGMI_SLOT();
        oc[1] = mfma_h(vb_h[1], pl[1], oc[1]);
        split_pm(st, 0, 0);
        PGMI_SLOT();
        oc[1] = mfma_h(vb_l[1], ph[1], oc[1]);
        split_pm(st, 0, 1);
        PGMI_SLOT();
        om[1] = mfma_h(vb_h[1], ph[1], om[1]);
        kfrag(Kb, 1, k1h, k1l);
        split_pm(st, 0, 2);
        PGMI_SLOT();
        sc = mfma_h(k0h, ql[0], zero16);
        split_pm(st, 0, 3);
        PGMI_SLOT();
        sc = mfma_h(k0l, qh[0], sc);
        split_pm(st, 1, 0);
        PGMI_SLOT();
        sm = mfma_h(k0h, qh[0], zero16);
        kfrag(Kb, 2, k0h, k0l);
        split_pm(st, 1, 1);
        PGMI_SLOT();
        sc = mfma_h(k1h, ql[1], sc);
        split_pm(st, 1, 2);
        PGMI_SLOT();
        sc = mfma_h(k1l, qh[1], sc);
        split_pm(st, 1, 3);
        PGMI_SLOT();
        sm = mfma_h(k1h, qh[1], sm);
        kfrag(Kb, 3, k1h, k1l);
        PGMI_SLOT();
        const bool dma_on = kt + 3 <= last_bundle;
        auto dma_slot = [&](int j) {
#pragma unroll
            for (int i = j; i < NDMA; i += 6) issue_piece(i, kt + 3, dma_stage, dma_on);
        };
        sc = mfma_h(k0h, ql[2], sc);
        dma_slot(0);
        PGMI_SLOT();
        sc = mfma_h(k0l, qh[2], sc);
        dma_slot(1);
        PGMI_SLOT();
        sm = mfma_h(k0h, qh[2], sm);
        dma_slot(2);
        PGMI_SLOT();
        sc = mfma_h(k1h, ql[3], sc);
        dma_slot(3);
        PGMI_SLOT();
        sc = mfma_h(k1l, qh[3], sc);
        dma_slot(4);
        PGMI_SLOT();
        sm = mfma_h(k1h, qh[3], sm);
        dma_slot(5);
#undef PGMI_SLOT
    };
    auto closing_pv = [&](const u32x4* stage) {
        apply_pending();
        const u32x4* Vb = stage + 2 * KCH;
        u32x4 va_h[ND], va_l[ND], vb_h[ND], vb_l[ND];
        vfrag(Vb, 0, va_h, va_l);
        vfrag(Vb, 1, vb_h, vb_l);
        pv(0, va_h, va_l);
        pv(1, vb_h, vb_l);
    };
    using T1 = std::integral_constant<bool, true>;
    using T0 = std::integral_constant<bool, false>;

    if (active && nkt > 0) {
#pragma unroll
        for (int s = 0; s < NS; ++s) {
            const int ci = r * KCPR + ((2 * s + kh) ^ k_swizzle<DH>(r));
            const u32x4 kfh = lds[ci], kfl = lds[KCH + ci];
            sc = mfma_h(kfh, ql[s], s == 0 ? zero16 : sc);
            sc = mfma_h(kfl, qh[s], sc);
            sm = mfma_h(kfh, qh[s], s == 0 ? zero16 : sm);
        }
    }
    auto wait_bundle = [&](int younger) {
        if (younger >= 1) asm volatile("s_waitcnt vmcnt(%0)" ::"n"(NDMA) : "memory");
        else asm volatile("s_waitcnt vmcnt(0)" ::: "memory");
    };
    int cur = 1;
    auto step_head = [&](int kt) {
        wait_bundle(1);
        __builtin_amdgcn_s_barrier();
        asm volatile("" ::: "memory");
    };
    auto idle_dma = [&](int kt) {
        issue_bundle(kt + 3, cur == 0 ? NSTG - 1 : cur - 1, kt + 3 <= last_bundle);
    };
    for (int kt = 0; kt < nkt - 1; ++kt) {
        step_head(kt);
        if (active) step(T0{}, kt, lds + cur * STG_CH, cur == 0 ? NSTG - 1 : cur - 1);
        else idle_dma(kt);
        cur = (cur == NSTG - 1) ? 0 : cur + 1;
    }
    step_head(nkt - 1);
    if (active) step(T1{}, nkt - 1, lds + cur * STG_CH, cur == 0 ? NSTG - 1 : cur - 1);
    else idle_dma(nkt - 1);
    cur = (cur == NSTG - 1) ? 0 : cur + 1;
    asm volatile("s_waitcnt vmcnt(0)" ::: "memory");
    __builtin_amdgcn_s_barrier();
    asm volatile("" ::: "memory");
    if (active) closing_pv(lds + cur * STG_CH);

    if (active) {
        const float l_tot = l_run + __shfl_xor(l_run, 32);
        const float inv = 1.0f / l_tot;
        const bool row_ok = q0 + r < T;
        const size_t orow = (size_t)(b * T + min(q0 + r, T - 1));
        if (OUT == ATT_OUT_BF16) store_ctx_bf16<ND>(om, oc, inv, kInvLo, row_ok, ctx16 + orow * (size_t)D + (size_t)h * DH, kh);
        else if (OUT == ATT_OUT_SPLIT) store_ctx_split<ND>(om, oc, inv, kInvLo, row_ok, ctx16 + orow * (size_t)(2 * D) + (size_t)(ND * h) * 64, kh);
        else if (row_ok) store_ctx_f32<ND>(om, oc, inv, kInvLo, ctx + (size_t)(b * T + q0 + r) * D + (size_t)h * DH + 4 * kh);
    }
}

static int g_att_v3 = -1;
void att_v3_set_option(int value) { g_att_v3 = value; }
bool att_v3_serves(const AttLaunch& a) {
    if (g_att_v3 == 0 || a.conv || a.slopes || a.head_dim != 64) return false;
    return g_att_v3 > 0 || (a.T + 31) / 32 >= 7;
}

using Att16v3Kernel = decltype(&attention_f16x3_v3_kernel<4, ATT_OUT_F32>);
struct Att16v3Inst { int wpb, out; Att16v3Kernel fn; };
template <int WPB, int OUT>
static constexpr Att16v3Inst att16v3_inst() { return {WPB, OUT, attention_f16x3_v3_kernel<WPB, OUT>}; }
static const Att16v3Inst kAtt16v3[] = {
    att16v3_inst<1, ATT_OUT_F32>(),   att16v3_inst<2, ATT_OUT_F32>(),   att16v3_inst<4, ATT_OUT_F32>(),
    att16v3_inst<1, ATT_OUT_SPLIT>(), att16v3_inst<2, ATT_OUT_SPLIT>(), att16v3_inst<4, ATT_OUT_SPLIT>(),
    att16v3_inst<1, ATT_OUT_BF16>(),  att16v3_inst<2, ATT_OUT_BF16>(),  att16v3_inst<4, ATT_OUT_BF16>(),
};

int launch_att16v3(const AttLaunch& a, int wpb, dim3 grid, int dense_nblk) {
    constexpr size_t lds_bytes = (size_t)3 * (2 * AKT * 8 + 2 * 64 * 4) * 16;
    for (const Att16v3Inst& k : kAtt16v3) {
        if (k.wpb != wpb || k.out != a.out) continue;
        hipLaunchKernelGGL(k.fn, grid, dim3(wpb * 64), lds_bytes, a.stream, a.qk16, a.qk_plane, a.vt16, a.vt_plane, a.kv_len, a.T, a.H, (a.T + 31) / 32 * 32,
                           a.ctx, a.ctx16, dense_nblk, a.B);
        PGMI_HIP(hipGetLastError());
        return PGMI_OK;
    }
    set_error("attention_f16x3_v3: no kernel for %d waves, output %d", wpb, (int)a.out);
    return PGMI_EINVAL;
}

}
```

### proteingym_amd/csrc/common.h

```cpp
#pragma once
#include <hip/hip_runtime.h>
#include <stdint.h>
#include <stddef.h>

#include "../../include/pgmi.h"

namespace pgmi {

void set_error(const char* fmt, ...);

#define PGMI_HIP(expr)                                                                   \
    do {                                                                                 \
        hipError_t _e = (expr);                                                          \
        if (_e != hipSuccess) {                                                          \
            pgmi::set_error("%s failed: %s (%s:%d)", #expr, hipGetErrorString(_e),       \
                            __FILE__, __LINE__);                                         \
            return PGMI_EHIP;                                                            \
        }                                                                                \
    } while (0)

typedef float f32x4 __attribute__((ext_vector_type(4)));
typedef float f32x16 __attribute__((ext_vector_type(16)));

constexpr int kWave = 64;
constexpr int kHeadDim = 64;

enum Epilogue { EPI_NONE = 0, EPI_GELU = 1, EPI_SQRELU = 2, EPI_GELU_TANH = 3,
                EPI_SWIGLU = 4 };

constexpr float kLoScale = 2048.0f;
constexpr float kQLog2e = 1.4426950408889634f;

__host__ __device__ __forceinline__ size_t ki_off(size_t row, int k, int K) {
    return row * (size_t)(2 * K) + (size_t)(k >> 5) * 64 + (size_t)(k & 31);
}
#if defined(__HIPCC__)
__device__ __forceinline__ void split_act(float x, _Float16& hi, _Float16& lo) {
    hi = (fabsf(x) < 6.103515625e-05f) ? (_Float16)0.0f : (_Float16)x;
    lo = (_Float16)((x - (float)hi) * kLoScale);
}
#endif

void launch_make_masked_windows(const int32_t* wt, const int32_t* win_start, const int32_t* mask_rel,
                                int B, int T, int32_t* tokens_out, hipStream_t s);
void launch_apply_mask(int32_t* tokens, const int32_t* mask_pos, int B, int T, hipStream_t s);
void launch_seq_stats(const int32_t* tokens, int B, int T, int token_dropout, float* scale,
                      int32_t* pos_idx, int32_t* kv_len, hipStream_t s, int mask_id = PGMI_TOK_MASK);
void launch_zero_pad_rows(const int32_t* tokens, int rows, int D, float* x, hipStream_t s);
void launch_embed(const int32_t* tokens, const float* scale, const int32_t* pos_idx,
                  const float* embed_tokens, const float* embed_positions, int token_dropout,
                  int rows, int T, int D, float* x, hipStream_t s, int mask_id = PGMI_TOK_MASK);
void launch_layernorm(const float* x, const float* w, const float* b, int rows, int D, float eps,
                      float* y, hipStream_t s);
void launch_gather_rows(const float* x, const int32_t* row_idx, int n, int D, float* y, hipStream_t s);
void launch_strided_index(int first, int stride, int n, int32_t* idx, hipStream_t s);
void launch_vocab_logsoftmax(const float* h, const float* E, const float* bias, int rows, int D,
                             int V, float* out, int32_t* nonfinite, hipStream_t s);
void launch_layernorm16(const float* x, const float* w, const float* b, int rows, int D, float eps,
                        unsigned short* y16, size_t plane, int mode, hipStream_t s);
void launch_scatter_rows(const float* src, const int32_t* dst_row, int n, int V, float* table,
                         hipStream_t s);
void launch_row_index(const int32_t* mask_rel, int B, int T, int32_t* out, hipStream_t s);
void launch_fill_f32(float* p, int64_t n, float v, hipStream_t s);
void launch_seq_loglik(const float* lp, const int32_t* tokens, const int32_t* lens, int B, int T, int V,
                       const float* prior, const int32_t* a0, const int32_t* row0, const int32_t* n,
                       const int32_t* flip, float alpha, float* out, hipStream_t s);
void launch_seq_loglik_ragged(const float* lp, const int32_t* tokens, const int32_t* seq_off, const int32_t* seq_p,
                              const int32_t* seq_root, int B, int T, int V, const float* prior, const int32_t* a0,
                              const int32_t* row0, const int32_t* n, const int32_t* flip, float alpha, float* out, hipStream_t s);
void launch_pg2_seq_loglik(const float* lp, const int32_t* col, const int32_t* n_kept, int B, int T, int V, float* out, hipStream_t s);
void launch_embed_learned(const int32_t* tokens, const float* E, const float* P, int rows, int T, int D, float* x, hipStream_t s);
void launch_wide_logsoftmax(const float* logits, int ldl, int rows, int V, const int32_t* tgt, float* out, int32_t* nonfinite,
                            hipStream_t s);
void launch_seq_sum(const float* terms, const int32_t* off, int B, double* out, hipStream_t s);
void launch_score_mutants(const float* table, int V, const int32_t* sub_pos, const int32_t* sub_wt,
                          const int32_t* sub_mt, const int64_t* mut_off, int64_t n_mut,
                          double* scores, hipStream_t s);
void launch_rotary(float* qkv, const float* cos_t, const float* sin_t, int rows, int T, int H,
                   hipStream_t s, int rot_halves = 1);
void launch_make_pppl_rows(const uint8_t* tok8, const int64_t* seq_off, const int32_t* sid, const int64_t* rp, int J,
                           int64_t g0, int bc, int T, int32_t* tokens, int32_t* row_idx, int32_t* target, hipStream_t s);
void launch_pppl_pick(const float* lp, const int32_t* target, int bc, int V, float* terms, hipStream_t s);
void launch_pppl_sum(const float* terms, const int64_t* rp, const int32_t* sid, int J, int64_t first, double* out, hipStream_t s);
void launch_saprot_rows(const int32_t* wt, const int32_t* set_off, const int32_t* set_pos, int s0, int bc, int T, int first, int groups,
                        int width, int32_t* tokens, int32_t* keep, hipStream_t s);
int launch_group_logsoftmax(const float* h, const float* E, const float* bias, int rows, int D, int V, int first, int groups, int width,
                            float* full, float* group, int32_t* nonfinite, hipStream_t s);

enum EveTensor { PGMI_EVE_T_Z = 0, PGMI_EVE_T_KEEP = 1, PGMI_EVE_T_W = 16, PGMI_EVE_T_B = 32, PGMI_EVE_T_WOUT = 48, PGMI_EVE_T_BOUT = 49,
                 PGMI_EVE_T_CONV = 50, PGMI_EVE_T_SPARSITY = 51, PGMI_EVE_T_TEMP = 52 };
void launch_eve_gather(const uint8_t* res, const float* W0t, const float* b, int rows, int L, int ld, int act, float* out, hipStream_t s);
void launch_eve_act(float* x, int rows, int n, int ld, int act, uint32_t keep24, float scale, uint64_t seed, uint32_t sample, int tensor,
                    int64_t row_base, const uint8_t* inj, int64_t inj_row0, hipStream_t s);
void launch_eve_latent(const float* mulv, int ldz, int64_t mulv_row0, int rows, int z, int ld, uint32_t keep24, float scale, uint64_t seed,
                       uint32_t sample, int64_t row_base, const float* inj_eps, const uint8_t* inj_keep, int64_t inj_row0, float* h,
                       hipStream_t s);
void launch_eve_sample(const float* mean, const float* sd, int64_t n, int K, int Kp, uint64_t seed, uint32_t sample, int tensor,
                       const float* inj, float* out, hipStream_t s);
void launch_eve_sample_final(const float* w_mean, const float* w_sd, const float* c_mean, const float* c_sd, const float* s_mean,
                             const float* s_sd, int L, int H, int Hp, int C, int Ht, bool conv, uint64_t seed, uint32_t sample,
                             const float* inj_w, const float* inj_c, const float* inj_s, float* out, hipStream_t s);
void launch_eve_elbo(const float* logits, const uint8_t* res, const float* mulv, int ldz, int z, const float* temp, int rows, int L,
                     int64_t loc0, float* elbo, float* bce, float* kld, double* acc, int first, hipStream_t s);
void launch_eve_fill_normal(uint64_t seed, uint32_t sample, int tensor, uint64_t e0, int64_t n, float* out, hipStream_t s);
void launch_eve_fill_keep(uint64_t seed, uint32_t sample, int tensor, uint64_t e0, int64_t n, uint32_t keep24, uint8_t* out, hipStream_t s);
int eve_set_option(const char* name, long long value);

void launch_msa_window_tokens(const int32_t* full, int R, int Tfull, int start, int Tw, int mask_col, int32_t* out, hipStream_t s);
void launch_add_row_embedding(float* x, const float* pe, int R, int C, int D, hipStream_t s);
void launch_permute_rows(const float* src, float* dst, int A, int B, int D, hipStream_t s);
void launch_tied_prep_qk(const float* qkv, int64_t M, int D, unsigned short* q16, unsigned short* k16, hipStream_t s);
void launch_pack_vt16(const float* qkv, int R, int C, int Kp, int H, unsigned short* Vt, hipStream_t s);
int launch_tied_softmax16(const float* part, int H, int S, int C, int Kp, float scale, unsigned short* P, hipStream_t s);
float tied_w_scale();

int launch_gemm_f32(const float* A, const float* W, const float* bias, const float* residual,
                    float* C, int M, int N, int K, int epilogue, hipStream_t s);

void gemm_options_from_env();
int gemm_set_option(const char* name, long long value);
int launch_gemm16(const unsigned short* A, size_t a_plane, const unsigned short* W, size_t w_plane,
                  const float* bias, const float* residual, float* Cf, unsigned short* Ch, size_t c_plane,
                  int M, int N, int K, int epilogue, float out_scale, int planes, bool bf, int variant,
                  hipStream_t s);
int launch_gemm16_qkv(const unsigned short* A, size_t a_plane, const unsigned short* W, size_t w_plane,
                      const float* bias, int M, int D, int K, float out_scale, unsigned short* qk16, size_t qk_plane,
                      unsigned short* vt16, size_t vt_plane, const float* cos_t, const float* sin_t, int rotary,
                      int T, int H, int variant, hipStream_t s, int rot_halves = 1, bool bf = false);
struct XMap;
int launch_gemm16_ex(const unsigned short* A, const unsigned short* W, float* Cf, unsigned short* Ch, int M, int N, int K,
                     float out_scale, XMap xm, int nbatch, hipStream_t s);
void launch_split16(const float* x, int64_t n, float scale, int mode, int K, unsigned short* out, hipStream_t s);

int launch_qkln_prep(const float* qkv, const float* q_w, const float* k_w, float eps, const float* cos_t, const float* sin_t, int B,
                     int T, int H, unsigned short* qk16, size_t qk_plane, unsigned short* vt16, size_t vt_plane, hipStream_t s);

int launch_attention_f32(const float* qkv, const int32_t* kv_len, int B, int T, int H, float* ctx, hipStream_t s,
                         int head_dim = 64);

enum AttOut {
    ATT_OUT_F32 = 0,
    ATT_OUT_SPLIT = 1,
    ATT_OUT_BF16 = 2
};
struct AttLaunch {
    unsigned short* qk16 = nullptr;
    size_t qk_plane = 0;
    unsigned short* vt16 = nullptr;
    size_t vt_plane = 0;
    int B = 1, T = 0, H = 0;
    int head_dim = 64;
    const int32_t* kv_len = nullptr;
    const float* slopes = nullptr;
    AttOut out = ATT_OUT_F32;
    float* ctx = nullptr;
    unsigned short* ctx16 = nullptr;
    hipStream_t stream = nullptr;
    const float* qkv = nullptr;
    const float* conv = nullptr;
    const float* cos_t = nullptr;
    const float* sin_t = nullptr;
    int rotary = 0;
};
int launch_attention_f16x3_v2(const AttLaunch& a);

struct AttRagged {
    const int32_t* seq_off;
    const int32_t* seq_p;
    const int32_t* seq_q;
    const int32_t* seq_root;
    const uint32_t* seq_vt;
    const int32_t* tile_seq;
    const int32_t* tile_j;
    const int32_t* blk_seq;
    const int32_t* blk_j;
    int n_tiles, n_blocks;
};
int att16_waves_per_block(int T);
int att_set_option(const char* name, long long value);
int launch_attention_tr_ragged(const AttLaunch& a, const AttRagged& rg);

}
```

### proteingym_amd/csrc/elementwise.hip

```cpp
#include "common.h"

namespace pgmi {

__device__ __forceinline__ float wave_sum(float v) {
#pragma unroll
    for (int o = 32; o > 0; o >>= 1) v += __shfl_xor(v, o);
    return v;
}
__device__ __forceinline__ float wave_max(float v) {
#pragma unroll
    for (int o = 32; o > 0; o >>= 1) v = fmaxf(v, __shfl_xor(v, o));
    return v;
}
__device__ __forceinline__ double wave_sum_d(double v) {
#pragma unroll
    for (int o = 32; o > 0; o >>= 1) v += __shfl_xor(v, o);
    return v;
}
__device__ __forceinline__ int wave_sum_i(int v) {
#pragma unroll
    for (int o = 32; o > 0; o >>= 1) v += __shfl_xor(v, o);
    return v;
}

__global__ void make_masked_windows_kernel(const int32_t* __restrict__ wt,
                                           const int32_t* __restrict__ win_start,
                                           const int32_t* __restrict__ mask_rel, int B, int T,
                                           int32_t* __restrict__ out) {
    const int64_t i = (int64_t)blockIdx.x * blockDim.x + threadIdx.x;
    if (i >= (int64_t)B * T) return;
    const int b = (int)(i / T), t = (int)(i % T);
    out[i] = (t == mask_rel[b]) ? PGMI_TOK_MASK : wt[win_start[b] + t];
}
void launch_make_masked_windows(const int32_t* wt, const int32_t* win_start, const int32_t* mask_rel,
                                int B, int T, int32_t* out, hipStream_t s) {
    const int64_t n = (int64_t)B * T;
    hipLaunchKernelGGL(make_masked_windows_kernel, dim3((unsigned)((n + 255) / 256)), dim3(256), 0, s,
                       wt, win_start, mask_rel, B, T, out);
}

__global__ void apply_mask_kernel(int32_t* tokens, const int32_t* __restrict__ mask_pos, int B, int T) {
    const int b = blockIdx.x * blockDim.x + threadIdx.x;
    if (b < B) tokens[(int64_t)b * T + mask_pos[b]] = PGMI_TOK_MASK;
}
void launch_apply_mask(int32_t* tokens, const int32_t* mask_pos, int B, int T, hipStream_t s) {
    hipLaunchKernelGGL(apply_mask_kernel, dim3((B + 255) / 256), dim3(256), 0, s, tokens, mask_pos, B, T);
}

__global__ void seq_stats_kernel(const int32_t* __restrict__ tokens, int B, int T, int token_dropout, int mask_id,
                                 float* __restrict__ denom, int32_t* __restrict__ pos_idx,
                                 int32_t* __restrict__ kv_len) {
    const int b = blockIdx.x * (blockDim.x >> 6) + (threadIdx.x >> 6);
    const int lane = threadIdx.x & 63;
    if (b >= B) return;
    const int32_t* tk = tokens + (int64_t)b * T;
    int running = 0, n_mask = 0, last_valid = -1;
    for (int t0 = 0; t0 < T; t0 += 64) {
        const int t = t0 + lane;
        const int tok = (t < T) ? tk[t] : PGMI_TOK_PAD;
        const int valid = (t < T) && (tok != PGMI_TOK_PAD);
        const unsigned long long bal = __ballot(valid);
        const unsigned long long below = bal & ((lane == 63) ? ~0ull : ((1ull << (lane + 1)) - 1ull));
        const int incl = __popcll(below);
        if (t < T) pos_idx[(int64_t)b * T + t] = valid ? (running + incl + PGMI_TOK_PAD) : PGMI_TOK_PAD;
        running += __popcll(bal);
        n_mask += __popcll(__ballot((t < T) && tok == mask_id));
        if (bal) last_valid = t0 + 63 - __clzll(bal);
    }
    if (lane == 0) {
        float d = 1.0f;
        if (token_dropout) d = 1.0f - (float)n_mask / (float)running;
        denom[b] = d;
        kv_len[b] = last_valid + 1;
    }
}
void launch_seq_stats(const int32_t* tokens, int B, int T, int token_dropout, float* denom,
                      int32_t* pos_idx, int32_t* kv_len, hipStream_t s, int mask_id) {
    hipLaunchKernelGGL(seq_stats_kernel, dim3((B + 3) / 4), dim3(256), 0, s, tokens, B, T, token_dropout, mask_id,
                       denom, pos_idx, kv_len);
}

__global__ void embed_kernel(const int32_t* __restrict__ tokens, const float* __restrict__ denom,
                             const int32_t* __restrict__ pos_idx, const float* __restrict__ E,
                             const float* __restrict__ P, int token_dropout, int mask_id, int rows, int T, int D,
                             float* __restrict__ x) {
    const int row = blockIdx.x * (blockDim.x >> 6) + (threadIdx.x >> 6);
    const int lane = threadIdx.x & 63;
    if (row >= rows) return;
    const int tok = tokens[row];
    const int b = row / T;
    const float dn = denom[b];
    const f32x4* e = reinterpret_cast<const f32x4*>(E + (size_t)tok * D);
    const f32x4* p = P ? reinterpret_cast<const f32x4*>(P + (size_t)pos_idx[row] * D) : nullptr;
    f32x4* xo = reinterpret_cast<f32x4*>(x + (size_t)row * D);
    const bool is_pad = tok == PGMI_TOK_PAD;
    const bool zero_emb = token_dropout && tok == mask_id;
    for (int i = lane; i < D / 4; i += 64) {
        f32x4 v = zero_emb ? f32x4{0.f, 0.f, 0.f, 0.f} : e[i];
        if (token_dropout) {
#pragma unroll
            for (int c = 0; c < 4; ++c) v[c] = (v[c] * 0.88f) / dn;
        }
        if (p) {
            const f32x4 pv = p[i];
#pragma unroll
            for (int c = 0; c < 4; ++c) v[c] += pv[c];
        }
        if (is_pad) v = f32x4{0.f, 0.f, 0.f, 0.f};
        xo[i] = v;
    }
}
void launch_embed(const int32_t* tokens, const float* denom, const int32_t* pos_idx, const float* E,
                  const float* P, int token_dropout, int rows, int T, int D, float* x, hipStream_t s, int mask_id) {
    hipLaunchKernelGGL(embed_kernel, dim3((rows + 3) / 4), dim3(256), 0, s, tokens, denom, pos_idx, E, P,
                       token_dropout, mask_id, rows, T, D, x);
}

__global__ void zero_pad_rows_kernel(const int32_t* __restrict__ tokens, int rows, int D, float* __restrict__ x) {
    const int row = blockIdx.x * 4 + (threadIdx.x >> 6);
    const int lane = threadIdx.x & 63;
    if (row >= rows || tokens[row] != PGMI_TOK_PAD) return;
    for (int i = lane; i < D; i += 64) x[(size_t)row * D + i] = 0.f;
}
void launch_zero_pad_rows(const int32_t* tokens, int rows, int D, float* x, hipStream_t s) {
    hipLaunchKernelGGL(zero_pad_rows_kernel, dim3((rows + 3) / 4), dim3(256), 0, s, tokens, rows, D, x);
}

template <int NV, int OUTMODE>
__global__ __launch_bounds__(256) void layernorm_kernel(const float* x,
                                                        const float* __restrict__ w,
                                                        const float* __restrict__ bsh, int rows, int D,
                                                        float eps, float* y, unsigned short* y16,
                                                        size_t plane) {
    const int row = blockIdx.x * 4 + (threadIdx.x >> 6);
    const int lane = threadIdx.x & 63;
    if (row >= rows) return;
    const int nv = D >> 2;
    const f32x4* xr = reinterpret_cast<const f32x4*>(x + (size_t)row * D);
    f32x4 v[NV];
    float s = 0.f;
#pragma unroll
    for (int i = 0; i < NV; ++i) {
        const int c = lane + 64 * i;
        v[i] = (c < nv) ? xr[c] : f32x4{0.f, 0.f, 0.f, 0.f};
        s += (v[i][0] + v[i][1]) + (v[i][2] + v[i][3]);
    }
    const float mean = wave_sum(s) / (float)D;
    float q = 0.f;
#pragma unroll
    for (int i = 0; i < NV; ++i) {
        const int c = lane + 64 * i;
        if (c < nv) {
#pragma unroll
            for (int k = 0; k < 4; ++k) {
                const float d = v[i][k] - mean;
                q += d * d;
            }
        }
    }
    const float rstd = 1.0f / sqrtf(wave_sum(q) / (float)D + eps);
    const f32x4* wr = reinterpret_cast<const f32x4*>(w);
    const f32x4* br = reinterpret_cast<const f32x4*>(bsh);
#pragma unroll
    for (int i = 0; i < NV; ++i) {
        const int c = lane + 64 * i;
        if (c < nv) {
            const f32x4 wv = wr[c], bv = br[c];
            f32x4 o;
#pragma unroll
            for (int k = 0; k < 4; ++k) o[k] = (v[i][k] - mean) * rstd * wv[k] + bv[k];
            if constexpr (OUTMODE == 0) {
                reinterpret_cast<f32x4*>(y + (size_t)row * D)[c] = o;
            } else if constexpr (OUTMODE == 1) {
                typedef _Float16 h4 __attribute__((ext_vector_type(4)));
                h4 hi, lo;
#pragma unroll
                for (int k = 0; k < 4; ++k) {
                    _Float16 a, b2;
                    split_act(o[k], a, b2);
                    hi[k] = a;
                    lo[k] = b2;
                }
                typedef unsigned int u32x2 __attribute__((ext_vector_type(2)));
                typedef unsigned int u32x4 __attribute__((ext_vector_type(4)));
                const u32x2 H = __builtin_bit_cast(u32x2, hi), L = __builtin_bit_cast(u32x2, lo);
                const bool odd = lane & 1;
                const unsigned int s0 = odd ? H[0] : L[0], s1 = odd ? H[1] : L[1];
                const unsigned int r0 = __shfl_xor(s0, 1), r1 = __shfl_xor(s1, 1);
                const u32x4 out = odd ? u32x4{r0, r1, L[0], L[1]} : u32x4{H[0], H[1], r0, r1};
                unsigned short* dst = y16 + ki_off((size_t)row, 4 * (c & ~1), D) + (odd ? 32 : 0);
                *reinterpret_cast<u32x4*>(dst) = out;
            } else {
                typedef unsigned int u32x2 __attribute__((ext_vector_type(2)));
                unsigned short b[4];
#pragma unroll
                for (int k = 0; k < 4; ++k) {
                    const float ok = o[k];
                    unsigned int u = __builtin_bit_cast(unsigned int, ok);
                    u += 0x7fffu + ((u >> 16) & 1u);
                    b[k] = (unsigned short)(u >> 16);
                }
                u32x2 pk;
                pk[0] = b[0] | ((unsigned)b[1] << 16);
                pk[1] = b[2] | ((unsigned)b[3] << 16);
                reinterpret_cast<u32x2*>(y16 + (size_t)row * D)[c] = pk;
            }
        }
    }
}
template <int OUTMODE>
static void launch_ln_mode(const float* x, const float* w, const float* b, int rows, int D, float eps,
                           float* y, unsigned short* y16, size_t plane, hipStream_t s) {
    const dim3 grid((rows + 3) / 4), block(256);
    const int nv = (D / 4 + 63) / 64;
    if (nv <= 1) hipLaunchKernelGGL((layernorm_kernel<1, OUTMODE>), grid, block, 0, s, x, w, b, rows, D, eps, y, y16, plane);
    else if (nv <= 2) hipLaunchKernelGGL((layernorm_kernel<2, OUTMODE>), grid, block, 0, s, x, w, b, rows, D, eps, y, y16, plane);
    else if (nv <= 5) hipLaunchKernelGGL((layernorm_kernel<5, OUTMODE>), grid, block, 0, s, x, w, b, rows, D, eps, y, y16, plane);
    else if (nv <= 10) hipLaunchKernelGGL((layernorm_kernel<10, OUTMODE>), grid, block, 0, s, x, w, b, rows, D, eps, y, y16, plane);
    else hipLaunchKernelGGL((layernorm_kernel<20, OUTMODE>), grid, block, 0, s, x, w, b, rows, D, eps, y, y16, plane);
}
void launch_layernorm(const float* x, const float* w, const float* b, int rows, int D, float eps,
                      float* y, hipStream_t s) {
    launch_ln_mode<0>(x, w, b, rows, D, eps, y, nullptr, 0, s);
}
void launch_layernorm16(const float* x, const float* w, const float* b, int rows, int D, float eps,
                        unsigned short* y16, size_t plane, int mode, hipStream_t s) {
    if (mode == 1) launch_ln_mode<1>(x, w, b, rows, D, eps, nullptr, y16, plane, s);
    else launch_ln_mode<2>(x, w, b, rows, D, eps, nullptr, y16, plane, s);
}

__global__ void rotary_kernel(float* __restrict__ qkv, const float* __restrict__ cos_t,
                              const float* __restrict__ sin_t, int64_t n, int T, int H, int rh) {
    const int64_t i = (int64_t)blockIdx.x * blockDim.x + threadIdx.x;
    if (i >= n) return;
    const int d = (int)(i & 31);
    const int64_t j = i >> 5;
    const int h = (int)(j % H);
    const int64_t k2 = j / H;
    const int which = (int)(k2 & 1);
    const int64_t row = k2 >> 1;
    const int t = (int)(row % T);
    float* p = qkv + row * (size_t)(3 * H * 64) + (size_t)which * H * 64 + h * 64 + d;
    const float x1 = p[0], x2 = p[32];
    const int tr = (t * rh + (h % rh)) * 64;
    const float c1 = cos_t[tr + d], s1 = sin_t[tr + d];
    const float c2 = cos_t[tr + d + 32], s2 = sin_t[tr + d + 32];
    p[0] = x1 * c1 + (-x2) * s1;
    p[32] = x2 * c2 + x1 * s2;
}
void launch_rotary(float* qkv, const float* cos_t, const float* sin_t, int rows, int T, int H, hipStream_t s, int rot_halves) {
    const int64_t n = (int64_t)rows * 2 * H * 32;
    hipLaunchKernelGGL(rotary_kernel, dim3((unsigned)((n + 255) / 256)), dim3(256), 0, s, qkv, cos_t, sin_t, n, T, H, rot_halves);
}

__global__ void gather_rows_kernel(const float* __restrict__ x, const int32_t* __restrict__ idx, int n,
                                   int D, float* __restrict__ y) {
    const int row = blockIdx.x * 4 + (threadIdx.x >> 6);
    const int lane = threadIdx.x & 63;
    if (row >= n) return;
    const f32x4* src = reinterpret_cast<const f32x4*>(x + (size_t)idx[row] * D);
    f32x4* dst = reinterpret_cast<f32x4*>(y + (size_t)row * D);
    for (int i = lane; i < D / 4; i += 64) dst[i] = src[i];
}
void launch_gather_rows(const float* x, const int32_t* idx, int n, int D, float* y, hipStream_t s) {
    hipLaunchKernelGGL(gather_rows_kernel, dim3((n + 3) / 4), dim3(256), 0, s, x, idx, n, D, y);
}

__global__ void strided_index_kernel(int first, int stride, int n, int32_t* __restrict__ idx) {
    const int i = blockIdx.x * blockDim.x + threadIdx.x;
    if (i < n) idx[i] = first + i * stride;
}
void launch_strided_index(int first, int stride, int n, int32_t* idx, hipStream_t s) {
    hipLaunchKernelGGL(strided_index_kernel, dim3((n + 255) / 256), dim3(256), 0, s, first, stride, n, idx);
}

__global__ void scatter_rows_kernel(const float* __restrict__ src, const int32_t* __restrict__ dst_row,
                                    int n, int V, float* __restrict__ table) {
    const int i = blockIdx.x * blockDim.x + threadIdx.x;
    if (i >= n * V) return;
    const int rI = i / V, c = i % V;
    table[(size_t)dst_row[rI] * V + c] = src[i];
}
void launch_scatter_rows(const float* src, const int32_t* dst_row, int n, int V, float* table, hipStream_t s) {
    hipLaunchKernelGGL(scatter_rows_kernel, dim3((n * V + 255) / 256), dim3(256), 0, s, src, dst_row, n, V, table);
}

__global__ void row_index_kernel(const int32_t* __restrict__ mask_rel, int B, int T, int32_t* __restrict__ out) {
    const int b = blockIdx.x * blockDim.x + threadIdx.x;
    if (b < B) out[b] = b * T + mask_rel[b];
}
void launch_row_index(const int32_t* mask_rel, int B, int T, int32_t* out, hipStream_t s) {
    hipLaunchKernelGGL(row_index_kernel, dim3((B + 255) / 256), dim3(256), 0, s, mask_rel, B, T, out);
}

__global__ void fill_f32_kernel(float* p, int64_t n, float v) {
    const int64_t i = (int64_t)blockIdx.x * blockDim.x + threadIdx.x;
    if (i < n) p[i] = v;
}
void launch_fill_f32(float* p, int64_t n, float v, hipStream_t s) {
    hipLaunchKernelGGL(fill_f32_kernel, dim3((unsigned)((n + 255) / 256)), dim3(256), 0, s, p, n, v);
}

__global__ __launch_bounds__(256) void vocab_logsoftmax_kernel(const float* __restrict__ h,
                                                               const float* __restrict__ E,
                                                               const float* __restrict__ bias, int rows,
                                                               int D, int V, float* __restrict__ out,
                                                               int32_t* __restrict__ nonfinite) {
    const int row = blockIdx.x * 4 + (threadIdx.x >> 6);
    const int lane = threadIdx.x & 63;
    if (row >= rows) return;
    const float* hr = h + (size_t)row * D;
    double my_logit = -INFINITY;
    for (int v = 0; v < V; ++v) {
        const float* ev = E + (size_t)v * D;
        double acc = 0.0;
        for (int i = lane; i < D; i += 64) acc = fma((double)hr[i], (double)ev[i], acc);
        acc = wave_sum_d(acc);
        if (lane == v) my_logit = acc + (double)bias[v];
    }
    const float mx = wave_max((float)my_logit);
    const double ex = (lane < V) ? exp(my_logit - (double)mx) : 0.0;
    const double lse = log(wave_sum_d(ex));
    const float res = (float)((my_logit - (double)mx) - lse);
    if (lane < V) {
        out[(size_t)row * V + lane] = res;
        if (nonfinite && !(fabsf(res) <= 3.0e38f)) atomicOr(nonfinite, 1);
    }
}
void launch_vocab_logsoftmax(const float* h, const float* E, const float* bias, int rows, int D, int V,
                             float* out, int32_t* nonfinite, hipStream_t s) {
    hipLaunchKernelGGL(vocab_logsoftmax_kernel, dim3((rows + 3) / 4), dim3(256), 0, s, h, E, bias, rows, D, V, out, nonfinite);
}

__global__ __launch_bounds__(256) void seq_loglik_kernel(const float* __restrict__ lp, const int32_t* __restrict__ tokens,
                                                         const int32_t* __restrict__ lens, int B, int T, int V,
                                                         const float* __restrict__ prior, const int32_t* __restrict__ a0,
                                                         const int32_t* __restrict__ row0, const int32_t* __restrict__ n,
                                                         const int32_t* __restrict__ flip, float alpha,
                                                         float* __restrict__ out) {
    const int b = blockIdx.x * 4 + (threadIdx.x >> 6);
    const int lane = threadIdx.x & 63;
    if (b >= B) return;
    const int len = lens[b];
    float acc = 0.f;
    for (int t = lane; t < len - 1; t += 64) {
        const int tgt = tokens[(size_t)b * T + t + 1];
        float v = lp[((size_t)b * T + t) * V + tgt];
        if (prior && n[b] > 0 && t >= a0[b] && t < a0[b] + n[b]) {
            const int i = t - a0[b];
            const int row = flip[b] ? row0[b] + (n[b] - 1 - i) : row0[b] + i;
            v = (1.0f - alpha) * v + alpha * prior[(size_t)row * V + tgt];
        }
        acc += v;
    }
    acc = wave_sum(acc);
    if (lane == 0) out[b] = acc;
}
__global__ __launch_bounds__(256) void seq_loglik_ragged_kernel(const float* __restrict__ lp, const int32_t* __restrict__ tokens,
                                                                const int32_t* __restrict__ seq_off, const int32_t* __restrict__ seq_p,
                                                                const int32_t* __restrict__ seq_root, int B, int T, int V,
                                                                const float* __restrict__ prior, const int32_t* __restrict__ a0,
                                                                const int32_t* __restrict__ row0, const int32_t* __restrict__ n,
                                                                const int32_t* __restrict__ flip, float alpha,
                                                                float* __restrict__ out) {
    const int b = blockIdx.x * 4 + (threadIdx.x >> 6);
    const int lane = threadIdx.x & 63;
    if (b >= B) return;
    const int a = seq_p[b], own0 = seq_off[b] - a, root0 = seq_off[seq_root[b]];
    float acc = 0.f;
    for (int t = lane; t < T - 1; t += 64) {
        const int tgt = tokens[(t + 1 < a) ? root0 + t + 1 : own0 + t + 1];
        float v = lp[(size_t)((t < a) ? root0 + t : own0 + t) * V + tgt];
        if (prior && n[b] > 0 && t >= a0[b] && t < a0[b] + n[b]) {
            const int i = t - a0[b];
            const int row = flip[b] ? row0[b] + (n[b] - 1 - i) : row0[b] + i;
            v = (1.0f - alpha) * v + alpha * prior[(size_t)row * V + tgt];
        }
        acc += v;
    }
    acc = wave_sum(acc);
    if (lane == 0) out[b] = acc;
}
void launch_seq_loglik_ragged(const float* lp, const int32_t* tokens, const int32_t* seq_off, const int32_t* seq_p,
                              const int32_t* seq_root, int B, int T, int V, const float* prior, const int32_t* a0,
                              const int32_t* row0, const int32_t* n, const int32_t* flip, float alpha, float* out, hipStream_t s) {
    hipLaunchKernelGGL(seq_loglik_ragged_kernel, dim3((B + 3) / 4), dim3(256), 0, s, lp, tokens, seq_off, seq_p, seq_root, B, T, V,
                       prior, a0, row0, n, flip, alpha, out);
}
void launch_seq_loglik(const float* lp, const int32_t* tokens, const int32_t* lens, int B, int T, int V,
                       const float* prior, const int32_t* a0, const int32_t* row0, const int32_t* n,
                       const int32_t* flip, float alpha, float* out, hipStream_t s) {
    hipLaunchKernelGGL(seq_loglik_kernel, dim3((B + 3) / 4), dim3(256), 0, s, lp, tokens, lens, B, T, V, prior, a0, row0, n,
                       flip, alpha, out);
}

__global__ __launch_bounds__(256) void pg2_seq_loglik_kernel(const float* __restrict__ lp, const int32_t* __restrict__ col,
                                                             const int32_t* __restrict__ n_kept, int B, int T, int V,
                                                             float* __restrict__ out) {
    const int b = blockIdx.x * 4 + (threadIdx.x >> 6);
    const int lane = threadIdx.x & 63;
    if (b >= B) return;
    const int n = n_kept[b];
    double acc = 0.0;
    for (int t = lane; t < n; t += 64) acc += (double)lp[((size_t)b * T + t) * V + col[(size_t)b * T + t]];
    acc = wave_sum_d(acc);
    if (lane == 0) out[b] = (float)acc;
}
void launch_pg2_seq_loglik(const float* lp, const int32_t* col, const int32_t* n_kept, int B, int T, int V, float* out, hipStream_t s) {
    hipLaunchKernelGGL(pg2_seq_loglik_kernel, dim3((B + 3) / 4), dim3(256), 0, s, lp, col, n_kept, B, T, V, out);
}

__global__ void score_mutants_kernel(const float* __restrict__ table, int V,
                                     const int32_t* __restrict__ sub_pos,
                                     const int32_t* __restrict__ sub_wt,
                                     const int32_t* __restrict__ sub_mt,
                                     const int64_t* __restrict__ mut_off, int64_t n_mut,
                                     double* __restrict__ scores) {
    const int64_t i = (int64_t)blockIdx.x * blockDim.x + threadIdx.x;
    if (i >= n_mut) return;
    double sc = 0.0;
    for (int64_t k = mut_off[i]; k < mut_off[i + 1]; ++k) {
        const float* rowp = table + (size_t)sub_pos[k] * V;
        const float d = rowp[sub_mt[k]] - rowp[sub_wt[k]];
        sc += (double)d;
    }
    scores[i] = sc;
}
void launch_score_mutants(const float* table, int V, const int32_t* sub_pos, const int32_t* sub_wt,
                          const int32_t* sub_mt, const int64_t* mut_off, int64_t n_mut, double* scores,
                          hipStream_t s) {
    if (n_mut <= 0) return;
    hipLaunchKernelGGL(score_mutants_kernel, dim3((unsigned)((n_mut + 255) / 256)), dim3(256), 0, s, table, V,
                       sub_pos, sub_wt, sub_mt, mut_off, n_mut, scores);
}


__global__ __launch_bounds__(256) void make_pppl_rows_kernel(const uint8_t* __restrict__ tok8, const int64_t* __restrict__ seq_off,
                                                             const int32_t* __restrict__ sid, const int64_t* __restrict__ rp, int J,
                                                             int64_t g0, int bc, int T, int32_t* __restrict__ tokens,
                                                             int32_t* __restrict__ row_idx, int32_t* __restrict__ target) {
    const int b = blockIdx.x * 4 + (threadIdx.x >> 6);
    const int lane = threadIdx.x & 63;
    if (b >= bc) return;
    const int64_t g = g0 + b;
    int lo = 0, hi = J;
    while (hi - lo > 1) {
        const int mid = (lo + hi) >> 1;
        if (rp[mid] <= g) lo = mid; else hi = mid;
    }
    const int n = sid[lo];
    const int i = 1 + (int)(g - rp[lo]);
    const int64_t o = seq_off[n];
    const int len = (int)(seq_off[n + 1] - o);
    int32_t* out = tokens + (int64_t)b * T;
    for (int t = lane; t < T; t += 64) out[t] = (t == i) ? PGMI_TOK_MASK : (t < len ? (int32_t)tok8[o + t] : PGMI_TOK_PAD);
    if (lane == 0) {
        row_idx[b] = b * T + i;
        target[b] = (int32_t)tok8[o + i + 1];
    }
}
void launch_make_pppl_rows(const uint8_t* tok8, const int64_t* seq_off, const int32_t* sid, const int64_t* rp, int J,
                           int64_t g0, int bc, int T, int32_t* tokens, int32_t* row_idx, int32_t* target, hipStream_t s) {
    hipLaunchKernelGGL(make_pppl_rows_kernel, dim3((bc + 3) / 4), dim3(256), 0, s, tok8, seq_off, sid, rp, J, g0, bc, T,
                       tokens, row_idx, target);
}

__global__ void pppl_pick_kernel(const float* __restrict__ lp, const int32_t* __restrict__ target, int bc, int V,
                                 float* __restrict__ terms) {
    const int b = blockIdx.x * blockDim.x + threadIdx.x;
    if (b < bc) terms[b] = lp[(size_t)b * V + target[b]];
}
void launch_pppl_pick(const float* lp, const int32_t* target, int bc, int V, float* terms, hipStream_t s) {
    hipLaunchKernelGGL(pppl_pick_kernel, dim3((bc + 255) / 256), dim3(256), 0, s, lp, target, bc, V, terms);
}

__global__ void pppl_sum_kernel(const float* __restrict__ terms, const int64_t* __restrict__ rp, const int32_t* __restrict__ sid,
                                int J, int64_t first, double* __restrict__ out) {
    const int j = blockIdx.x * blockDim.x + threadIdx.x;
    if (j >= J) return;
    double acc = 0.0;
    for (int64_t g = rp[j]; g < rp[j + 1]; ++g) acc += (double)terms[g];
    out[sid[j] - first] = acc;
}
void launch_pppl_sum(const float* terms, const int64_t* rp, const int32_t* sid, int J, int64_t first, double* out, hipStream_t s) {
    if (J <= 0) return;
    hipLaunchKernelGGL(pppl_sum_kernel, dim3((J + 127) / 128), dim3(128), 0, s, terms, rp, sid, J, first, out);
}


__global__ __launch_bounds__(256) void embed_learned_kernel(const int32_t* __restrict__ tokens, const float* __restrict__ E,
                                                            const float* __restrict__ P, int rows, int T, int D, float* __restrict__ x) {
    const int row = blockIdx.x * 4 + (threadIdx.x >> 6);
    const int lane = threadIdx.x & 63;
    if (row >= rows) return;
    const f32x4* e = reinterpret_cast<const f32x4*>(E + (size_t)tokens[row] * D);
    const f32x4* p = reinterpret_cast<const f32x4*>(P + (size_t)(row % T) * D);
    f32x4* xo = reinterpret_cast<f32x4*>(x + (size_t)row * D);
    for (int i = lane; i < D / 4; i += 64) xo[i] = e[i] + p[i];
}
void launch_embed_learned(const int32_t* tokens, const float* E, const float* P, int rows, int T, int D, float* x, hipStream_t s) {
    hipLaunchKernelGGL(embed_learned_kernel, dim3((rows + 3) / 4), dim3(256), 0, s, tokens, E, P, rows, T, D, x);
}

__device__ __forceinline__ void lse_merge(float& m, double& s, float m2, double s2) {
    const float M = fmaxf(m, m2);
    const double a = s == 0.0 ? 0.0 : s * exp((double)m - (double)M);
    const double b = s2 == 0.0 ? 0.0 : s2 * exp((double)m2 - (double)M);
    m = M;
    s = a + b;
}
__global__ __launch_bounds__(256) void wide_logsoftmax_kernel(const float* __restrict__ logits, int ldl, int V,
                                                              const int32_t* __restrict__ tgt, float* __restrict__ out,
                                                              int32_t* __restrict__ nonfinite) {
    __shared__ float sm[256];
    __shared__ double ss[256];
    const int r = blockIdx.x, tid = threadIdx.x;
    const float* row = logits + (size_t)r * ldl;
    const f32x4* row4 = reinterpret_cast<const f32x4*>(row);
    float m = -INFINITY;
    double s = 0.0;
    for (int i = tid; i < (V + 3) / 4; i += 256) {
        const f32x4 v = row4[i];
        const int c0 = 4 * i;
        float mx = m;
#pragma unroll
        for (int k = 0; k < 4; ++k)
            if (c0 + k < V) mx = fmaxf(mx, v[k]);
        if (mx > m) {
            s = s == 0.0 ? 0.0 : s * (double)__expf(m - mx);
            m = mx;
        }
        float e = 0.0f;
#pragma unroll
        for (int k = 0; k < 4; ++k)
            if (c0 + k < V) e += __expf(v[k] - m);
        s += (double)e;
    }
    sm[tid] = m;
    ss[tid] = s;
    __syncthreads();
    for (int o = 128; o > 0; o >>= 1) {
        if (tid < o) {
            float a = sm[tid];
            double b = ss[tid];
            lse_merge(a, b, sm[tid + o], ss[tid + o]);
            sm[tid] = a;
            ss[tid] = b;
        }
        __syncthreads();
    }
    const double lse = (double)sm[0] + log(ss[0]);
    bool bad = false;
    if (tgt) {
        if (tid == 0) {
            const float res = (float)((double)row[tgt[r]] - lse);
            out[r] = res;
            bad = !(fabsf(res) <= 3.0e38f);
        }
    } else {
        for (int c = tid; c < V; c += 256) {
            const float res = (float)((double)row[c] - lse);
            out[(size_t)r * V + c] = res;
            bad |= !(fabsf(res) <= 3.0e38f);
        }
    }
    if (nonfinite && bad) atomicOr(nonfinite, 1);
}
void launch_wide_logsoftmax(const float* logits, int ldl, int rows, int V, const int32_t* tgt, float* out, int32_t* nonfinite,
                            hipStream_t s) {
    if (rows <= 0) return;
    hipLaunchKernelGGL(wide_logsoftmax_kernel, dim3(rows), dim3(256), 0, s, logits, ldl, V, tgt, out, nonfinite);
}

__global__ void seq_sum_kernel(const float* __restrict__ terms, const int32_t* __restrict__ off, int B, double* __restrict__ out) {
    const int b = blockIdx.x * blockDim.x + threadIdx.x;
    if (b >= B) return;
    double acc = 0.0;
    for (int i = off[b]; i < off[b + 1]; ++i) acc += (double)terms[i];
    out[b] = acc;
}
void launch_seq_sum(const float* terms, const int32_t* off, int B, double* out, hipStream_t s) {
    hipLaunchKernelGGL(seq_sum_kernel, dim3((B + 127) / 128), dim3(128), 0, s, terms, off, B, out);
}

__global__ __launch_bounds__(256) void saprot_rows_kernel(const int32_t* __restrict__ wt, const int32_t* __restrict__ set_off,
                                                          const int32_t* __restrict__ set_pos, int s0, int bc, int T, int first,
                                                          int groups, int width, int32_t* __restrict__ tokens,
                                                          int32_t* __restrict__ keep) {
    const int b = blockIdx.x * 4 + (threadIdx.x >> 6);
    const int lane = threadIdx.x & 63;
    if (b >= bc) return;
    const int e0 = set_off[s0], lo0 = set_off[s0 + b], hi0 = set_off[s0 + b + 1];
    int32_t* out = tokens + (int64_t)b * T;
    for (int t = lane; t < T; t += 64) {
        int lo = lo0, hi = hi0;
        while (lo < hi) {
            const int mid = (lo + hi) >> 1;
            if (set_pos[mid] < t) lo = mid + 1; else hi = mid;
        }
        const int id = wt[t];
        const bool masked = lo < hi0 && set_pos[lo] == t && id >= first;
        out[t] = masked ? first + (groups - 1) * width + (id - first) % width : id;
    }
    for (int e = lo0 + lane; e < hi0; e += 64) keep[e - e0] = b * T + set_pos[e];
}
void launch_saprot_rows(const int32_t* wt, const int32_t* set_off, const int32_t* set_pos, int s0, int bc, int T, int first, int groups,
                        int width, int32_t* tokens, int32_t* keep, hipStream_t s) {
    hipLaunchKernelGGL(saprot_rows_kernel, dim3((bc + 3) / 4), dim3(256), 0, s, wt, set_off, set_pos, s0, bc, T, first, groups, width,
                       tokens, keep);
}

constexpr int kGroupSlots = 8;
template <int NV>
__global__ __launch_bounds__(256) void group_logsoftmax_kernel(const float* __restrict__ h, const float* __restrict__ E,
                                                               const float* __restrict__ bias, int rows, int D, int V, int first,
                                                               int groups, int width, float* __restrict__ full,
                                                               float* __restrict__ group, int32_t* __restrict__ nonfinite) {
    const int row = blockIdx.x * 4 + (threadIdx.x >> 6);
    const int lane = threadIdx.x & 63;
    if (row >= rows) return;
    const int nv = D >> 2;
    const f32x4* hr = reinterpret_cast<const f32x4*>(h + (size_t)row * D);
    f32x4 x[NV];
#pragma unroll
    for (int i = 0; i < NV; ++i) {
        const int c = lane + 64 * i;
        x[i] = (c < nv) ? hr[c] : f32x4{0.f, 0.f, 0.f, 0.f};
    }
    double lg[kGroupSlots];
#pragma unroll
    for (int j = 0; j < kGroupSlots; ++j) {
        lg[j] = -INFINITY;
        for (int l = 0; l < 64; ++l) {
            const int v = 64 * j + l;
            if (v >= V) break;
            const f32x4* ev = reinterpret_cast<const f32x4*>(E + (size_t)v * D);
            double acc = 0.0;
#pragma unroll
            for (int i = 0; i < NV; ++i) {
                const int c = lane + 64 * i;
                if (c < nv) {
                    const f32x4 e = ev[c];
#pragma unroll
                    for (int k = 0; k < 4; ++k) acc = fma((double)x[i][k], (double)e[k], acc);
                }
            }
            acc = wave_sum_d(acc);
            if (lane == l) lg[j] = acc + (double)bias[v];
        }
    }
    float mx = -INFINITY;
#pragma unroll
    for (int j = 0; j < kGroupSlots; ++j) mx = fmaxf(mx, (float)lg[j]);
    mx = wave_max(mx);
    double ex = 0.0;
#pragma unroll
    for (int j = 0; j < kGroupSlots; ++j) ex += (64 * j + lane < V) ? exp(lg[j] - (double)mx) : 0.0;
    const double lse = (double)mx + log(wave_sum_d(ex));
    bool bad = false;
    if (full) {
#pragma unroll
        for (int j = 0; j < kGroupSlots; ++j) {
            const int v = 64 * j + lane;
            if (v < V) {
                const float res = (float)(lg[j] - lse);
                full[(size_t)row * V + v] = res;
                bad |= !(fabsf(res) <= 3.0e38f);
            }
        }
    }
    if (group) {
        float mine = 0.f;
        for (int g = 0; g < groups; ++g) {
            const int c0 = first + g * width;
            double val = -INFINITY;
#pragma unroll
            for (int j = 0; j < kGroupSlots; ++j) {
                const int v = 64 * j + lane;
                if (v >= c0 && v < c0 + width && v < V) val = lg[j];
            }
            const float gm = wave_max((float)val);
            const double gs = wave_sum_d(val == -INFINITY ? 0.0 : exp(val - (double)gm));
            const float res = (float)(((double)gm + log(gs)) - lse);
            if (lane == g) mine = res;
        }
        if (lane < groups) {
            group[(size_t)row * groups + lane] = mine;
            bad |= !(fabsf(mine) <= 3.0e38f);
        }
    }
    if (nonfinite && bad) atomicOr(nonfinite, 1);
}
int launch_group_logsoftmax(const float* h, const float* E, const float* bias, int rows, int D, int V, int first, int groups, int width,
                            float* full, float* group, int32_t* nonfinite, hipStream_t s) {
    if (rows <= 0) return PGMI_OK;
    const int nv = (D / 4 + 63) / 64;
    if (D % 4 || nv > 10 || V > 64 * kGroupSlots || groups > 64 || width > 64 || first + groups * width > V) {
        set_error("grouped log-softmax: unsupported shape (D %d, V %d, %d groups of %d from column %d)", D, V, groups, width, first);
        return PGMI_EINVAL;
    }
    const dim3 grid((rows + 3) / 4), block(256);
#define PGMI_GLS(N) hipLaunchKernelGGL((group_logsoftmax_kernel<N>), grid, block, 0, s, h, E, bias, rows, D, V, first, groups, width, full, group, nonfinite)
    if (nv <= 1) PGMI_GLS(1); else if (nv <= 2) PGMI_GLS(2); else if (nv <= 5) PGMI_GLS(5); else PGMI_GLS(10);
#undef PGMI_GLS
    return PGMI_OK;
}

}
```

### proteingym_amd/csrc/model.h

```cpp
#pragma once
#include <math.h>
#include <stdlib.h>
#include <cmath>
#include <algorithm>
#include <stdarg.h>
#include <stdio.h>
#include <string.h>

#include <string>
#include <vector>

#include "common.h"
#include "gemm16x_kernel.h"

namespace pgmi {

struct W16 {
    unsigned short* p = nullptr;
    size_t plane = 0;
    float out_scale = 1.0f;
};

struct Layer {
    float *ln1_w, *ln1_b, *wqkv, *bqkv, *wo, *bo, *ln2_w, *ln2_b, *w1, *b1, *w2, *b2;
    W16 wqkv16, wo16, w116, w216;
    float* conv = nullptr;
    float *c_ln_w = nullptr, *c_ln_b = nullptr, *c_bqkv = nullptr, *c_bo = nullptr;
    W16 c_wqkv16, c_wo16;
    float *q_ln = nullptr, *k_ln = nullptr;
};

struct ProfEvent {
    hipEvent_t start, stop;
    int cls;
};

}

using namespace pgmi;

struct pgmi_assay;
struct pgmi_pppl;

struct pgmi_model {
    pgmi_config cfg;
    int device = 0;
    hipStream_t stream = nullptr;
    std::vector<void*> allocs;
    std::vector<pgmi_assay*> assays;
    std::vector<pgmi_pppl*> pppls;
    float *embed_tokens = nullptr, *embed_positions = nullptr;
    float *lnb_w = nullptr, *lnb_b = nullptr, *lna_w = nullptr, *lna_b = nullptr;
    float *hd_w = nullptr, *hd_b = nullptr, *hln_w = nullptr, *hln_b = nullptr;
    float *head_w = nullptr, *head_b = nullptr;
    std::vector<Layer> layers;
    W16 hd16;
    int fc1_epi = EPI_GELU, fc1_cols = 0;
    bool embed_gather = false;
    int mask_id = PGMI_TOK_MASK, n_token_ids = PGMI_VOCAB;
    float* slopes = nullptr;
    float* tr_prior = nullptr;
    size_t tr_prior_cap = 0;
    int32_t* tr_meta = nullptr;
    size_t tr_meta_cap = 0;
    int pg2_rotary = 0;
    float *pg2_aa_w = nullptr, *pg2_aa_b = nullptr;
    int gpt_Vp = 0, gpt_head_rows = 0;
    bool parallel_residual = false;
    float* gpt_logits = nullptr;
    W16 gpt_head16;
    double* gpt_sum = nullptr;
    float* msa_pe = nullptr;
    float* xt = nullptr;
    int32_t *msa_full = nullptr, *msa_kv_len = nullptr;
    size_t msa_full_cap = 0;
    float *tied_part = nullptr, *tied_p = nullptr, *tied_vt = nullptr;
    size_t tied_part_cap = 0, tied_p_cap = 0, tied_vt_cap = 0;
    int msa_kv_R = 0, msa_kv_C = 0;
    float ln_eps = 1e-5f;
    unsigned short *h16 = nullptr, *g16 = nullptr;
    size_t h16_plane = 0, g16_plane = 0;
    unsigned short *qk16 = nullptr, *vt16 = nullptr;
    size_t qk16_plane = 0, vt16_plane = 0;
    int32_t* nonfinite = nullptr;
    int gemm_variant = 0;
    int keep_rows = 1;
    int last_B = 0, last_T = 0;
    int dh = kHeadDim;
    int rot_halves = 1;
    int Hs = 0;
    int Da = 0;
    float *rot_cos = nullptr, *rot_sin = nullptr;
    int rot_len = 0;
    float* zeros = nullptr;
    int max_rows = 0;
    float *x = nullptr, *h = nullptr, *qkv = nullptr, *g = nullptr, *lp = nullptr, *denom = nullptr;
    int32_t *tokens = nullptr, *pos_idx = nullptr, *kv_len = nullptr, *row_idx = nullptr, *aux_i = nullptr;
    bool prof = false;
    std::vector<ProfEvent> events;
    size_t events_used = 0;
    double prof_ms[PGMI_K_COUNT] = {0};
    int64_t prof_n[PGMI_K_COUNT] = {0};
    double prof_flops[PGMI_K_COUNT] = {0};
    double prof_bytes[PGMI_K_COUNT] = {0};
};

struct pgmi_assay {
    pgmi_model* m = nullptr;
    int n_tok = 0, P = 0, T = 0;
    int64_t n_mut = 0, n_sub = 0;
    std::vector<void*> allocs;
    int32_t *wt = nullptr, *positions = nullptr, *win_start = nullptr, *mask_rel = nullptr;
    int32_t *sub_pos = nullptr, *sub_wt = nullptr, *sub_mt = nullptr;
    int64_t* mut_off = nullptr;
    float* table = nullptr;
    double* scores = nullptr;
};

struct pgmi_pppl {
    pgmi_model* m = nullptr;
    int64_t N = 0;
    std::vector<int64_t> off;
    std::vector<void*> allocs;
    uint8_t* tok8 = nullptr;
    int64_t* off_dev = nullptr;
    int64_t last_rows = 0, last_chunks = 0, last_tokens = 0, last_padded = 0;
};

namespace pgmi {

template <typename T>
int dev_alloc(std::vector<void*>& pool, T** p, size_t n) {
    void* q = nullptr;
    if (n == 0) n = 1;
    hipError_t e = hipMalloc(&q, n * sizeof(T));
    if (e != hipSuccess) {
        set_error("hipMalloc(%zu bytes) failed: %s", n * sizeof(T), hipGetErrorString(e));
        return PGMI_ENOMEM;
    }
    pool.push_back(q);
    *p = static_cast<T*>(q);
    return PGMI_OK;
}

template <typename T>
int dev_upload(std::vector<void*>& pool, T** p, const T* host, size_t n) {
    int rc = dev_alloc(pool, p, n);
    if (rc) return rc;
    if (n) PGMI_HIP(hipMemcpy(*p, host, n * sizeof(T), hipMemcpyHostToDevice));
    return PGMI_OK;
}

struct ProfScope {
    pgmi_model* m;
    ProfEvent* ev = nullptr;
    ProfScope(pgmi_model* m_, int cls, double flops, double bytes) : m(m_) {
        if (!m->prof) return;
        if (m->events_used == m->events.size()) {
            ProfEvent e;
            if (hipEventCreate(&e.start) != hipSuccess || hipEventCreate(&e.stop) != hipSuccess) return;
            m->events.push_back(e);
        }
        ev = &m->events[m->events_used++];
        ev->cls = cls;
        m->prof_n[cls] += 1;
        m->prof_flops[cls] += flops;
        m->prof_bytes[cls] += bytes;
        hipEventRecord(ev->start, m->stream);
    }
    ~ProfScope() {
        if (ev) hipEventRecord(ev->stop, m->stream);
    }
};

template <typename T>
int ensure_cap(pgmi_model* m, T** p, size_t* cap, size_t need) {
    if (need <= *cap) return PGMI_OK;
    T* q = nullptr;
    int rc = dev_alloc(m->allocs, &q, need);
    if (rc) return rc;
    *p = q;
    *cap = need;
    return PGMI_OK;
}

int prof_drain(pgmi_model* m);
int check_cfg(const pgmi_config* c);
int check_tokens(const int32_t* tokens, int B, int T, int n_ids = PGMI_VOCAB);
int check_vocab(const int32_t* tokens, int B, int T, int V);
int env_int(const char* name, int dflt);
int make_w16(std::vector<void*>& pool, const float* host, size_t n, size_t K, int precision, hipStream_t s, W16* out);
int linear(pgmi_model* m, const float* in32, const unsigned short* in16, size_t in_plane, const float* W32,
           const W16& w16, const float* bias, const float* residual, float* out32, unsigned short* out16,
           size_t out_plane, int M, int N, int K, int epi);
int check_nonfinite(pgmi_model* m);
int reset_pad_keys(pgmi_model* m, int B, int T);
int model_create(const pgmi_config* cfg, const float* w, int64_t n_weights, int device, pgmi_model** out, int arch_arg);
int create_esm(pgmi_model* m, const pgmi_config* cfg, const float* w, int64_t n_weights);
int ensure_rotary(pgmi_model* m, int T);
int upload_rotate_half(pgmi_model* m, int n);
int run_encoder(pgmi_model* m, int B, int T, const int32_t* keep = nullptr, int n_keep = 0, bool* compacted = nullptr);
int head_hidden(pgmi_model* m, int R, const int32_t* row_idx);
int run_head(pgmi_model* m, int R, const int32_t* row_idx);
int run_rows(pgmi_model* m, int B, int T, int R, const int32_t* row_idx);
int create_tranception(pgmi_model* m, const pgmi_config* cfg, const float* w, int64_t n_weights);
int create_progen2(pgmi_model* m, const pgmi_config* cfg, const float* w, int64_t n_weights, int rotary_dim);
int create_gpt(pgmi_model* m, const pgmi_config* cfg, const float* w, int64_t n_weights, int pos_kind);
int64_t gpt_weight_count(const pgmi_config* c, int pos_kind);
int decoder_check(pgmi_model* m, int arch, int T);
int run_decoder(pgmi_model* m, int B, int T, const AttRagged* rg = nullptr, int rows = 0, double att_flops = 0);
int narrow_head(pgmi_model* m, int M);
int decoder_token_logprobs(pgmi_model* m, int arch, const int32_t* tokens, int B, int T, float* out);
int64_t esmc_weight_count(const pgmi_config* c);
int create_esmc(pgmi_model* m, const pgmi_config* cfg, const float* w, int64_t n_weights);
int create_saprot(pgmi_model* m, const pgmi_config* cfg, const float* w, int64_t n_weights, int mask_id);
int create_msa(pgmi_model* m, const pgmi_config* cfg, const float* w, int64_t n_weights);
int run_msa(pgmi_model* m, int R, int C, int keep_col = -1, bool* compacted = nullptr);

inline bool esm2_rotary(int arch) { return arch == PGMI_ARCH_ESM2 || arch == PGMI_ARCH_SAPROT; }

struct BlobCursor {
    pgmi_model* m;
    const float *p, *end;
    int rc = PGMI_OK;
    BlobCursor(pgmi_model* m_, const float* w, int64_t n_weights) : m(m_), p(w), end(w + n_weights) {}
    const float* take(size_t n) { p += n; return p - n; }
    void upload(float** dst, const float* host, size_t n) { if (!rc) rc = dev_upload(m->allocs, dst, host, n); }
    void upload(float** dst, size_t n) { upload(dst, take(n), n); }
    void w16(W16* dst, const float* host, size_t n, size_t K) { if (!rc) rc = make_w16(m->allocs, host, n, K, m->cfg.precision, m->stream, dst); }
    void w16(W16* dst, size_t n, size_t K) { w16(dst, take(n), n, K); }
    void linear(float** w32, W16* w16_, const float* host, size_t n, size_t K) {
        if (m->cfg.precision == PGMI_PREC_FP32) upload(w32, host, n); else w16(w16_, host, n, K);
    }
    void linear(float** w32, W16* w16_, size_t n, size_t K) { linear(w32, w16_, take(n), n, K); }
    int finish() {
        if (!rc && p != end) { set_error("internal: blob walk mismatch"); rc = PGMI_EINVAL; }
        return rc;
    }
};

inline size_t rotate_half_slot(size_t col, size_t dh) {
    const size_t h = col / dh, j = col % dh;
    if (dh > 64) return (2 * h + ((j >> 5) & 1)) * 64 + ((j >> 6) << 5) + (j & 31);
    return h * 64 + (j < dh / 2 ? j : 32 + (j - dh / 2));
}

template <typename Slot>
void pack_qkv_slots(const float* src, size_t D, size_t Da, Slot slot, float qscale, float* wq, float* bq = nullptr) {
    for (size_t k = 0; k < 3; ++k) {
        const float sc = (k == 0) ? qscale : 1.0f;
        for (size_t o = 0; o < D; ++o) {
            float* dst = &wq[(k * Da + slot(o)) * D];
            for (size_t i = 0; i < D; ++i) dst[i] = src[o * D + i] * sc;
        }
        src += D * D;
        if (!bq) continue;
        for (size_t o = 0; o < D; ++o) bq[k * Da + slot(o)] = src[o] * sc;
        src += D;
    }
}

template <typename Slot>
void pack_out_cols(const float* src, size_t D, size_t Da, Slot slot, float* wo) {
    for (size_t o = 0; o < D; ++o)
        for (size_t i = 0; i < D; ++i) wo[o * Da + slot(i)] = src[o * D + i];
}

template <typename Angle>
int upload_rotary(pgmi_model* m, int n, int groups, Angle angle) {
    std::vector<float> c((size_t)n * groups * 64), s((size_t)n * groups * 64);
    for (int t = 0; t < n; ++t)
        for (int g = 0; g < groups; ++g)
            for (int i = 0; i < 32; ++i) {
                const float f = angle(t, g, i);
                const size_t o = ((size_t)t * groups + g) * 64;
                c[o + i] = c[o + 32 + i] = cosf(f);
                s[o + i] = s[o + 32 + i] = sinf(f);
            }
    int rc = dev_upload(m->allocs, &m->rot_cos, c.data(), c.size());
    if (!rc) rc = dev_upload(m->allocs, &m->rot_sin, s.data(), s.size());
    if (!rc) m->rot_len = n;
    return rc;
}

inline int rows_per_chunk(const pgmi_model* m, int T) { return std::max(1, m->max_rows / ((T + 31) / 32 * 32)); }

template <typename Fn>
int for_each_chunk(pgmi_model* m, int B, int T, Fn fn) {
    const int per = rows_per_chunk(m, T);
    for (int b0 = 0; b0 < B; b0 += per) {
        int rc = fn(b0, std::min(per, B - b0));
        if (rc) return rc;
        PGMI_HIP(hipStreamSynchronize(m->stream));
    }
    return PGMI_OK;
}

}
```

Baseline: 18510.

## Share layer-0 QKV across same-window masked rows and skip unneeded attention blocks

After: 18640, median of 6. No clear change (+0.7%).

```diff
diff --git a/proteingym_amd/csrc/api_esm.hip b/proteingym_amd/csrc/api_esm.hip
--- a/proteingym_amd/csrc/api_esm.hip
+++ b/proteingym_amd/csrc/api_esm.hip
@@ -59,7 +59,7 @@
     });
 }
 
-int run_encoder(pgmi_model* m, int B, int T, const int32_t* keep, int n_keep, bool* compacted) {
+int run_encoder(pgmi_model* m, int B, int T, const int32_t* keep, int n_keep, bool* compacted, const Layer0Share* share) {
     const pgmi_config& c = m->cfg;
     const int M = B * T, D = c.embed_dim, F = c.ffn_dim, N1 = m->fc1_cols, H = c.heads, Da = m->Da;
     hipStream_t s = m->stream;
@@ -85,6 +85,23 @@
     const int mode16 = (prec == PGMI_PREC_F16X3) ? 1 : 2;
     for (int l = 0; l < c.layers; ++l) {
         const Layer& L = m->layers[l];
+        const int Tp = (T + 31) / 32 * 32;
+        if (l == 0 && share && m->share_layer0 && prec != PGMI_PREC_FP32 && !L.q_ln && share->G > 0 && 4 * share->G <= B &&
+            (size_t)B * Tp <= (size_t)m->max_rows) {
+            const int Mc = 2 * share->G * T;
+            const size_t cqk_plane = (size_t)Mc * 2 * Da, cvt_plane = (size_t)2 * share->G * Da * Tp;
+            unsigned short* cqk = reinterpret_cast<unsigned short*>(m->qkv);
+            unsigned short* cvt = cqk + 2 * cqk_plane;
+            ProfScope p(m, PGMI_K_GEMM_QKV, 2.0 * Mc * 3 * D * D, 4.0 * ((double)M * 2 * Da + (double)M * Da));
+            launch_gather_rows(m->x, share->src_rows, Mc, D, m->g, s);
+            launch_layernorm16(m->g, L.ln1_w, L.ln1_b, Mc, D, 1e-5f, m->h16, m->h16_plane, mode16, s);
+            rc = launch_gemm16_qkv(m->h16, m->h16_plane, L.wqkv16.p, L.wqkv16.plane, L.bqkv, Mc, Da, D, L.wqkv16.out_scale,
+                                   cqk, cqk_plane, cvt, cvt_plane, m->rot_cos, m->rot_sin,
+                                   esm2_rotary(c.arch), T, m->Hs, m->gemm_variant, s, m->rot_halves, prec == PGMI_PREC_BF16);
+            if (rc) return rc;
+            launch_share_operands(cqk, cqk_plane, cvt, cvt_plane, share->seq_group, share->mask_rel, B, T, m->Hs,
+                                  m->qk16, m->qk16_plane, m->vt16, m->vt16_plane, s);
+        } else {
         { ProfScope p(m, PGMI_K_LAYERNORM, 0, ln_bytes);
           if (prec == PGMI_PREC_FP32) launch_layernorm(m->x, L.ln1_w, L.ln1_b, M, D, 1e-5f, m->h, s);
           else launch_layernorm16(m->x, L.ln1_w, L.ln1_b, M, D, 1e-5f, m->h16, m->h16_plane, mode16, s); }
@@ -97,11 +114,16 @@
           else
               rc = linear(m, m->h, m->h16, m->h16_plane, L.wqkv, L.wqkv16, L.bqkv, nullptr, m->qkv, nullptr, 0, M, 3 * Da, D, EPI_NONE);
           if (rc) return rc; }
-        { ProfScope p(m, PGMI_K_ATTENTION, 4.0 * M * T * D, L.q_ln ? (double)M * D * 20 : 0);
+        }
+        const bool v2 = prec != PGMI_PREC_FP32;
+        const int att_wpb = att16_waves_per_block(T), att_nblk = ((T + 31) / 32 + att_wpb - 1) / att_wpb;
+        const bool need_blocks = keep && m->keep_rows >= 2 && l == c.layers - 1 && v2 && m->rot_halves == 1 &&
+                                 (size_t)B * att_nblk <= (size_t)m->max_rows / 32 + 1;
+        const double att_share = need_blocks ? std::min(1.0, (double)n_keep / ((double)B * att_nblk)) : 1.0;
+        { ProfScope p(m, PGMI_K_ATTENTION, 4.0 * M * T * D * att_share, L.q_ln ? (double)M * D * 20 : 0);
           if (L.q_ln && (rc = launch_qkln_prep(m->qkv, L.q_ln, L.k_ln, 1e-5f, m->rot_cos, m->rot_sin, B, T, H, m->qk16, m->qk16_plane,
                                                m->vt16, m->vt16_plane, s)))
               return rc;
-          const bool v2 = prec != PGMI_PREC_FP32;
           if (esm2_rotary(c.arch) && !v2) launch_rotary(m->qkv, m->rot_cos, m->rot_sin, M, T, m->Hs, s, m->rot_halves);
           if (v2) {
               AttLaunch a;
@@ -111,6 +133,10 @@
               a.out = prec == PGMI_PREC_F16X3 ? ATT_OUT_SPLIT : ATT_OUT_BF16;
               a.ctx16 = m->h16;
               a.stream = s;
+              if (need_blocks) {
+                  launch_need_blocks(keep, n_keep, T, att_wpb * 32, att_nblk, m->att_need, (size_t)B * att_nblk, s);
+                  a.need = m->att_need;
+              }
               rc = launch_attention_f16x3_v2(a);
           } else {
               rc = launch_attention_f32(m->qkv, m->kv_len, B, T, H, m->h, s, m->rot_halves * kHeadDim);
@@ -185,11 +211,51 @@
 }
 
 
-int run_rows(pgmi_model* m, int B, int T, int R, const int32_t* row_idx) {
+int run_rows(pgmi_model* m, int B, int T, int R, const int32_t* row_idx, const Layer0Share* share) {
     bool compacted = false;
-    int rc = run_encoder(m, B, T, row_idx, R, &compacted);
+    int rc = run_encoder(m, B, T, row_idx, R, &compacted, share);
     if (rc) return rc;
     return run_head(m, R, compacted ? nullptr : row_idx);
+}
+
+static int build_layer0_share(pgmi_assay* a, const std::vector<int32_t>& ws, const std::vector<int32_t>& mr, int per) {
+    const int P = a->P, T = a->T;
+    std::vector<int32_t> group(P), src;
+    for (int p0 = 0; p0 < P; p0 += per) {
+        const int bc = std::min(per, P - p0);
+        std::vector<int32_t> start;
+        std::vector<std::vector<int32_t>> members;
+        for (int b = 0; b < bc; ++b) {
+            size_t g = std::find(start.begin(), start.end(), ws[p0 + b]) - start.begin();
+            if (g == start.size()) { start.push_back(ws[p0 + b]); members.emplace_back(); }
+            members[g].push_back(b);
+            group[p0 + b] = (int32_t)g;
+        }
+        const int G = (int)start.size();
+        a->share_G.push_back(G);
+        a->share_src_off.push_back(src.size());
+        const size_t base = src.size();
+        src.resize(base + (size_t)G * 2 * T);
+        for (int g = 0; g < G; ++g) {
+            int32_t* wt = &src[base + (size_t)g * 2 * T];
+            int32_t* mk = wt + T;
+            std::vector<int32_t> masked_at(T, -1);
+            for (int32_t b : members[g])
+                if (masked_at[mr[p0 + b]] < 0) masked_at[mr[p0 + b]] = b;
+            for (int t = 0; t < T; ++t) {
+                int32_t w = -1;
+                for (int32_t b : members[g])
+                    if (mr[p0 + b] != t) { w = b * T + t; break; }
+                const int32_t k = masked_at[t] >= 0 ? masked_at[t] * T + t : -1;
+                if (w < 0) w = k;
+                wt[t] = w;
+                mk[t] = k >= 0 ? k : w;
+            }
+        }
+    }
+    int rc = dev_upload(a->allocs, &a->share_group, group.data(), group.size());
+    if (!rc) rc = dev_upload(a->allocs, &a->share_src, src.data(), src.size());
+    return rc;
 }
 
 }
@@ -281,6 +347,7 @@
     if (!rc) rc = dev_upload(a->allocs, &a->mut_off, mut_off, (size_t)(n_mut + 1));
     if (!rc) rc = dev_alloc(a->allocs, &a->table, (size_t)n_tok * PGMI_VOCAB);
     if (!rc) rc = dev_alloc(a->allocs, &a->scores, (size_t)n_mut);
+    if (!rc) rc = build_layer0_share(a, ws, mr, rows_per_chunk(m, T));
     if (rc) { pgmi_assay_destroy(a); return rc; }
     m->assays.push_back(a);
     *out = a;
@@ -306,11 +373,16 @@
     const int T = a->T, V = m->cfg.vocab;
     const int per = rows_per_chunk(m, T);
     launch_fill_f32(a->table, (int64_t)a->n_tok * V, NAN, s);
-    for (int p0 = 0; p0 < a->P; p0 += per) {
+    for (int p0 = 0, chunk = 0; p0 < a->P; p0 += per, ++chunk) {
         const int bc = std::min(per, a->P - p0);
         launch_make_masked_windows(a->wt, a->win_start + p0, a->mask_rel + p0, bc, T, m->tokens, s);
         launch_row_index(a->mask_rel + p0, bc, T, m->row_idx, s);
-        int rc = run_rows(m, bc, T, bc, m->row_idx);
+        Layer0Share share;
+        share.G = a->share_G[chunk];
+        share.seq_group = a->share_group + p0;
+        share.mask_rel = a->mask_rel + p0;
+        share.src_rows = a->share_src + a->share_src_off[chunk];
+        int rc = run_rows(m, bc, T, bc, m->row_idx, &share);
         if (rc) return rc;
         launch_scatter_rows(m->lp, a->positions + p0, bc, V, a->table, s);
     }
diff --git a/proteingym_amd/csrc/api_model.hip b/proteingym_amd/csrc/api_model.hip
--- a/proteingym_amd/csrc/api_model.hip
+++ b/proteingym_amd/csrc/api_model.hip
@@ -247,6 +247,7 @@
         m->vt16_plane = R * Da;
         alloc(&m->qk16, m->qk16_plane * 2);
         alloc(&m->vt16, m->vt16_plane * 2);
+        alloc(&m->att_need, R / 32 + 1);
     }
     if (c.arch == PGMI_ARCH_MSA) {
         alloc(&m->xt, R * D);
@@ -305,7 +306,8 @@
     }
     if (!rc) rc = alloc_workspace(m);
     if (rc) { pgmi_model_destroy(m); return rc; }
-    m->keep_rows = env_int("PGMI_KEEP_ROWS", 1);
+    m->keep_rows = env_int("PGMI_KEEP_ROWS", 2);
+    m->share_layer0 = env_int("PGMI_SHARE_LAYER0", 1);
     gemm_options_from_env();
     m->gemm_variant = env_int("PGMI_GEMM_VARIANT", 0);
     *out = m;
diff --git a/proteingym_amd/csrc/attention_f16.hip b/proteingym_amd/csrc/attention_f16.hip
--- a/proteingym_amd/csrc/attention_f16.hip
+++ b/proteingym_amd/csrc/attention_f16.hip
@@ -6,11 +6,12 @@
 
 namespace pgmi {
 
-template <int WPB, int OUT, int NSTG, int DH = 64, bool RAG = false, int DO = DH>
+template <int WPB, int OUT, int NSTG, int DH = 64, bool RAG = false, int DO = DH, bool NEED = false>
 __global__ __launch_bounds__(WPB * 64) void attention_f16x3_v2_kernel(
     const unsigned short* __restrict__ qk16, size_t qk_plane, const unsigned short* __restrict__ vt16,
     size_t vt_plane, const int32_t* __restrict__ kv_len, const float* __restrict__ slopes, int T, int H,
-    int Tp, float* __restrict__ ctx, unsigned short* __restrict__ ctx16, RagMap rag, int dense_nblk, int nseq) {
+    int Tp, float* __restrict__ ctx, unsigned short* __restrict__ ctx16, RagMap rag, int dense_nblk, int nseq,
+    const unsigned char* __restrict__ need) {
     constexpr float defer_thr = kAttDefer;
     constexpr int NT = WPB * 64;
     constexpr int KCPR = DH / 8;
@@ -38,6 +39,10 @@
         b = blockIdx.z;
         hs = blockIdx.y;
         qblk_dense = blockIdx.x;
+    }
+    if constexpr (NEED) {
+        static_assert(!RAG && NSL == 1, "needed-block lists: dense launches of whole heads");
+        if (!need[b * (dense_nblk > 0 ? dense_nblk : (int)gridDim.x) + qblk_dense]) return;
     }
     h = hs / NSL;
     const int d0 = (hs - h * NSL) * DO;
@@ -274,10 +279,10 @@
 
 
 using Att16v2Kernel = decltype(&attention_f16x3_v2_kernel<4, ATT_OUT_F32, 3, 64, false, 64>);
-struct Att16v2Inst { int wpb, out, head_dim; bool rag; Att16v2Kernel fn; size_t lds_bytes; };
-template <int WPB, int OUT, int NSTG, int DH, bool RAG = false, int DO = DH>
+struct Att16v2Inst { int wpb, out, head_dim; bool rag, need; Att16v2Kernel fn; size_t lds_bytes; };
+template <int WPB, int OUT, int NSTG, int DH, bool RAG = false, int DO = DH, bool NEED = false>
 static constexpr Att16v2Inst att16v2_inst() {
-    return {WPB, OUT, DH, RAG, attention_f16x3_v2_kernel<WPB, OUT, NSTG, DH, RAG, DO>, (size_t)NSTG * (8 * DH + 8 * DO) * 16};
+    return {WPB, OUT, DH, RAG, NEED, attention_f16x3_v2_kernel<WPB, OUT, NSTG, DH, RAG, DO, NEED>, (size_t)NSTG * (8 * DH + 8 * DO) * 16};
 }
 static const Att16v2Inst kAtt16v2[] = {
     att16v2_inst<1, ATT_OUT_F32, 3, 64>(),   att16v2_inst<2, ATT_OUT_F32, 3, 64>(),   att16v2_inst<4, ATT_OUT_F32, 3, 64>(),
@@ -286,21 +291,24 @@
     att16v2_inst<1, ATT_OUT_SPLIT, 3, 64, true>(), att16v2_inst<2, ATT_OUT_SPLIT, 3, 64, true>(), att16v2_inst<4, ATT_OUT_SPLIT, 3, 64, true>(),
     att16v2_inst<4, ATT_OUT_F32, 3, 128>(),  att16v2_inst<4, ATT_OUT_SPLIT, 3, 128>(), att16v2_inst<4, ATT_OUT_BF16, 3, 128>(),
     att16v2_inst<4, ATT_OUT_SPLIT, 2, 256, false, 128>(),
+    att16v2_inst<1, ATT_OUT_SPLIT, 3, 64, false, 64, true>(), att16v2_inst<2, ATT_OUT_SPLIT, 3, 64, false, 64, true>(), att16v2_inst<4, ATT_OUT_SPLIT, 3, 64, false, 64, true>(),
+    att16v2_inst<1, ATT_OUT_BF16, 3, 64, false, 64, true>(),  att16v2_inst<2, ATT_OUT_BF16, 3, 64, false, 64, true>(),  att16v2_inst<4, ATT_OUT_BF16, 3, 64, false, 64, true>(),
 };
 
 static int launch_att16v2(const AttLaunch& a, int wpb, dim3 grid, const RagMap* rag, int dense_nblk) {
     for (const Att16v2Inst& k : kAtt16v2) {
-        if (k.wpb != wpb || k.out != a.out || k.head_dim != a.head_dim || k.rag != (rag != nullptr)) continue;
+        if (k.wpb != wpb || k.out != a.out || k.head_dim != a.head_dim || k.rag != (rag != nullptr) || k.need != (a.need != nullptr)) continue;
         if (k.lds_bytes > 65536) {
             hipError_t e = hipFuncSetAttribute(reinterpret_cast<const void*>(k.fn), hipFuncAttributeMaxDynamicSharedMemorySize, (int)k.lds_bytes);
             if (e != hipSuccess) { set_error("hipFuncSetAttribute: %s", hipGetErrorString(e)); return PGMI_EHIP; }
         }
         hipLaunchKernelGGL(k.fn, grid, dim3(wpb * 64), k.lds_bytes, a.stream, a.qk16, a.qk_plane, a.vt16, a.vt_plane, a.kv_len, a.slopes,
-                           a.T, a.H, (a.T + 31) / 32 * 32, a.ctx, a.ctx16, rag ? *rag : RagMap{}, dense_nblk, a.B);
+                           a.T, a.H, (a.T + 31) / 32 * 32, a.ctx, a.ctx16, rag ? *rag : RagMap{}, dense_nblk, a.B, a.need);
         PGMI_HIP(hipGetLastError());
         return PGMI_OK;
     }
-    set_error("attention_f16x3_v2: no kernel for %d waves, output %d, head_dim %d%s", wpb, (int)a.out, a.head_dim, rag ? ", ragged" : "");
+    set_error("attention_f16x3_v2: no kernel for %d waves, output %d, head_dim %d%s%s", wpb, (int)a.out, a.head_dim, rag ? ", ragged" : "",
+              a.need ? ", needed blocks" : "");
     return PGMI_EINVAL;
 }
 
@@ -344,6 +352,10 @@
     const int n32 = (T + 31) / 32, Tp = n32 * 32;
     int rc = check_operand_range("attention_f16x3_v2", a);
     if (rc) return rc;
+    if (a.need && (head_dim != 64 || a.slopes || a.conv || a.out == ATT_OUT_F32)) {
+        set_error("attention_f16x3_v2: a needed-block list goes with the dense head_dim 64 launch and 16-bit context rows only");
+        return PGMI_EINVAL;
+    }
     int dn = 0;
     if (head_dim == 256) {
         if (a.qkv || a.conv || !a.slopes || a.out != ATT_OUT_SPLIT) { set_error("attention_f16x3_v2: head_dim 256 is the causal, fused-QKV, split-plane-output flavour only"); return PGMI_EINVAL; }
diff --git a/proteingym_amd/csrc/attention_f16_v3.hip b/proteingym_amd/csrc/attention_f16_v3.hip
--- a/proteingym_amd/csrc/attention_f16_v3.hip
+++ b/proteingym_amd/csrc/attention_f16_v3.hip
@@ -6,11 +6,11 @@
 
 namespace pgmi {
 
-template <int WPB, int OUT>
+template <int WPB, int OUT, bool NEED = false>
 __global__ __launch_bounds__(WPB * 64, 2) void attention_f16x3_v3_kernel(
     const unsigned short* __restrict__ qk16, size_t qk_plane, const unsigned short* __restrict__ vt16, size_t vt_plane,
     const int32_t* __restrict__ kv_len, int T, int H, int Tp, float* __restrict__ ctx, unsigned short* __restrict__ ctx16,
-    int dense_nblk, int nseq) {
+    int dense_nblk, int nseq, const unsigned char* __restrict__ need) {
     constexpr float defer_thr = kAttDefer;
     constexpr int DH = 64, NSTG = 3, KCPR = 8, KCH = AKT * KCPR, VCH = DH * 4, STG_CH = 2 * KCH + 2 * VCH;
     constexpr int NWI = STG_CH / 64, NDMA = (NWI + WPB - 1) / WPB, NS = 4, ND = 2;
@@ -25,6 +25,9 @@
         b = blockIdx.z;
         h = blockIdx.y;
         qblk = blockIdx.x;
+    }
+    if constexpr (NEED) {
+        if (!need[b * (dense_nblk > 0 ? dense_nblk : (int)gridDim.x) + qblk]) return;
     }
     const int tid = threadIdx.x, lane = tid & 63;
     const int wave = __builtin_amdgcn_readfirstlane(tid >> 6);
@@ -361,25 +364,27 @@
 }
 
 using Att16v3Kernel = decltype(&attention_f16x3_v3_kernel<4, ATT_OUT_F32>);
-struct Att16v3Inst { int wpb, out; Att16v3Kernel fn; };
-template <int WPB, int OUT>
-static constexpr Att16v3Inst att16v3_inst() { return {WPB, OUT, attention_f16x3_v3_kernel<WPB, OUT>}; }
+struct Att16v3Inst { int wpb, out; bool need; Att16v3Kernel fn; };
+template <int WPB, int OUT, bool NEED = false>
+static constexpr Att16v3Inst att16v3_inst() { return {WPB, OUT, NEED, attention_f16x3_v3_kernel<WPB, OUT, NEED>}; }
 static const Att16v3Inst kAtt16v3[] = {
     att16v3_inst<1, ATT_OUT_F32>(),   att16v3_inst<2, ATT_OUT_F32>(),   att16v3_inst<4, ATT_OUT_F32>(),
     att16v3_inst<1, ATT_OUT_SPLIT>(), att16v3_inst<2, ATT_OUT_SPLIT>(), att16v3_inst<4, ATT_OUT_SPLIT>(),
     att16v3_inst<1, ATT_OUT_BF16>(),  att16v3_inst<2, ATT_OUT_BF16>(),  att16v3_inst<4, ATT_OUT_BF16>(),
+    att16v3_inst<1, ATT_OUT_SPLIT, true>(), att16v3_inst<2, ATT_OUT_SPLIT, true>(), att16v3_inst<4, ATT_OUT_SPLIT, true>(),
+    att16v3_inst<1, ATT_OUT_BF16, true>(),  att16v3_inst<2, ATT_OUT_BF16, true>(),  att16v3_inst<4, ATT_OUT_BF16, true>(),
 };
 
 int launch_att16v3(const AttLaunch& a, int wpb, dim3 grid, int dense_nblk) {
     constexpr size_t lds_bytes = (size_t)3 * (2 * AKT * 8 + 2 * 64 * 4) * 16;
     for (const Att16v3Inst& k : kAtt16v3) {
-        if (k.wpb != wpb || k.out != a.out) continue;
+        if (k.wpb != wpb || k.out != a.out || k.need != (a.need != nullptr)) continue;
         hipLaunchKernelGGL(k.fn, grid, dim3(wpb * 64), lds_bytes, a.stream, a.qk16, a.qk_plane, a.vt16, a.vt_plane, a.kv_len, a.T, a.H, (a.T + 31) / 32 * 32,
-                           a.ctx, a.ctx16, dense_nblk, a.B);
+                           a.ctx, a.ctx16, dense_nblk, a.B, a.need);
         PGMI_HIP(hipGetLastError());
         return PGMI_OK;
     }
-    set_error("attention_f16x3_v3: no kernel for %d waves, output %d", wpb, (int)a.out);
+    set_error("attention_f16x3_v3: no kernel for %d waves, output %d%s", wpb, (int)a.out, a.need ? ", needed blocks" : "");
     return PGMI_EINVAL;
 }
 
diff --git a/proteingym_amd/csrc/common.h b/proteingym_amd/csrc/common.h
--- a/proteingym_amd/csrc/common.h
+++ b/proteingym_amd/csrc/common.h
@@ -53,6 +53,9 @@
 void launch_layernorm(const float* x, const float* w, const float* b, int rows, int D, float eps,
                       float* y, hipStream_t s);
 void launch_gather_rows(const float* x, const int32_t* row_idx, int n, int D, float* y, hipStream_t s);
+void launch_share_operands(const unsigned short* cqk, size_t cqk_plane, const unsigned short* cvt, size_t cvt_plane,
+                           const int32_t* seq_group, const int32_t* mask_rel, int B, int T, int Hs,
+                           unsigned short* qk16, size_t qk_plane, unsigned short* vt16, size_t vt_plane, hipStream_t s);
 void launch_strided_index(int first, int stride, int n, int32_t* idx, hipStream_t s);
 void launch_vocab_logsoftmax(const float* h, const float* E, const float* bias, int rows, int D,
                              int V, float* out, int32_t* nonfinite, hipStream_t s);
@@ -61,6 +64,7 @@
 void launch_scatter_rows(const float* src, const int32_t* dst_row, int n, int V, float* table,
                          hipStream_t s);
 void launch_row_index(const int32_t* mask_rel, int B, int T, int32_t* out, hipStream_t s);
+void launch_need_blocks(const int32_t* keep, int n_keep, int T, int rows_per_blk, int nblk, unsigned char* need, size_t n_need, hipStream_t s);
 void launch_fill_f32(float* p, int64_t n, float v, hipStream_t s);
 void launch_seq_loglik(const float* lp, const int32_t* tokens, const int32_t* lens, int B, int T, int V,
                        const float* prior, const int32_t* a0, const int32_t* row0, const int32_t* n,
@@ -152,6 +156,7 @@
     int head_dim = 64;
     const int32_t* kv_len = nullptr;
     const float* slopes = nullptr;
+    const unsigned char* need = nullptr;
     AttOut out = ATT_OUT_F32;
     float* ctx = nullptr;
     unsigned short* ctx16 = nullptr;
diff --git a/proteingym_amd/csrc/elementwise.hip b/proteingym_amd/csrc/elementwise.hip
--- a/proteingym_amd/csrc/elementwise.hip
+++ b/proteingym_amd/csrc/elementwise.hip
@@ -266,6 +266,66 @@
     hipLaunchKernelGGL(gather_rows_kernel, dim3((n + 3) / 4), dim3(256), 0, s, x, idx, n, D, y);
 }
 
+__global__ __launch_bounds__(256) void share_operands_kernel(
+    const unsigned short* __restrict__ cqk, size_t cqk_plane, const unsigned short* __restrict__ cvt, size_t cvt_plane,
+    const int32_t* __restrict__ seq_group, const int32_t* __restrict__ mask_rel, int B, int T, int Hs,
+    unsigned short* __restrict__ qk16, size_t qk_plane, unsigned short* __restrict__ vt16, size_t vt_plane) {
+    typedef unsigned int u32x4 __attribute__((ext_vector_type(4)));
+    typedef unsigned short us8 __attribute__((ext_vector_type(8)));
+    const int M = B * T, Da = Hs * 64, Tp = (T + 31) / 32 * 32;
+    const int tid = threadIdx.x;
+    if ((int)blockIdx.x < M) {
+        const int m = blockIdx.x, b = m / T, t = m - b * T;
+        const int ps = 2 * seq_group[b] + (t == mask_rel[b] ? 1 : 0);
+        const unsigned short* src = cqk + ((size_t)ps * T + t) * (size_t)(2 * Da);
+        unsigned short* dst = qk16 + (size_t)m * (size_t)(2 * Da);
+        for (int c = tid; c < Da / 4; c += 256) {
+            const u32x4 hi = *reinterpret_cast<const u32x4*>(src + c * 8);
+            const u32x4 lo = *reinterpret_cast<const u32x4*>(src + cqk_plane + c * 8);
+            *reinterpret_cast<u32x4*>(dst + c * 8) = hi;
+            *reinterpret_cast<u32x4*>(dst + qk_plane + c * 8) = lo;
+        }
+        return;
+    }
+    const int blk = (int)blockIdx.x - M, b = blk / Hs, hs = blk - b * Hs;
+    const int g = seq_group[b], tm = mask_rel[b], tk = tm & 31;
+    const int pm = (tm & ~31) + ((tk & 0x13) | ((tk & 4) << 1) | ((tk & 8) >> 1));
+    const int cpr = Tp / 8;
+    const size_t blk_halfs = (size_t)64 * Tp;
+    const unsigned short* wt = cvt + ((size_t)(2 * g) * Hs + hs) * blk_halfs;
+    const unsigned short* mk = cvt + ((size_t)(2 * g + 1) * Hs + hs) * blk_halfs;
+    unsigned short* dst = vt16 + ((size_t)b * Hs + hs) * blk_halfs;
+    for (int i = tid; i < 64 * cpr; i += 256) {
+        const int d = i / cpr, j = i - d * cpr;
+        const size_t o = (size_t)d * Tp + j * 8;
+        us8 hi = *reinterpret_cast<const us8*>(wt + o), lo = *reinterpret_cast<const us8*>(wt + cvt_plane + o);
+        if (j == (pm >> 3)) {
+            hi[pm & 7] = mk[(size_t)d * Tp + pm];
+            lo[pm & 7] = mk[cvt_plane + (size_t)d * Tp + pm];
+        }
+        if ((j >> 2) * 32 + 32 <= T) {
+            *reinterpret_cast<us8*>(dst + o) = hi;
+            *reinterpret_cast<us8*>(dst + vt_plane + o) = lo;
+        } else {
+#pragma unroll
+            for (int e = 0; e < 8; ++e) {
+                const int pk = (j * 8 + e) & 31;
+                const int t = (j >> 2) * 32 + ((pk & 0x13) | ((pk & 4) << 1) | ((pk & 8) >> 1));
+                if (t < T) {
+                    dst[o + e] = hi[e];
+                    dst[vt_plane + o + e] = lo[e];
+                }
+            }
+        }
+    }
+}
+void launch_share_operands(const unsigned short* cqk, size_t cqk_plane, const unsigned short* cvt, size_t cvt_plane,
+                           const int32_t* seq_group, const int32_t* mask_rel, int B, int T, int Hs,
+                           unsigned short* qk16, size_t qk_plane, unsigned short* vt16, size_t vt_plane, hipStream_t s) {
+    hipLaunchKernelGGL(share_operands_kernel, dim3((unsigned)(B * T + B * Hs)), dim3(256), 0, s, cqk, cqk_plane, cvt, cvt_plane,
+                       seq_group, mask_rel, B, T, Hs, qk16, qk_plane, vt16, vt_plane);
+}
+
 __global__ void strided_index_kernel(int first, int stride, int n, int32_t* __restrict__ idx) {
     const int i = blockIdx.x * blockDim.x + threadIdx.x;
     if (i < n) idx[i] = first + i * stride;
@@ -291,6 +351,18 @@
 }
 void launch_row_index(const int32_t* mask_rel, int B, int T, int32_t* out, hipStream_t s) {
     hipLaunchKernelGGL(row_index_kernel, dim3((B + 255) / 256), dim3(256), 0, s, mask_rel, B, T, out);
+}
+
+__global__ void need_blocks_kernel(const int32_t* __restrict__ keep, int n_keep, int T, int rows_per_blk, int nblk,
+                                   unsigned char* __restrict__ need) {
+    const int i = blockIdx.x * blockDim.x + threadIdx.x;
+    if (i >= n_keep) return;
+    const int b = keep[i] / T, t = keep[i] - b * T;
+    need[(size_t)b * nblk + t / rows_per_blk] = 1;
+}
+void launch_need_blocks(const int32_t* keep, int n_keep, int T, int rows_per_blk, int nblk, unsigned char* need, size_t n_need, hipStream_t s) {
+    (void)hipMemsetAsync(need, 0, n_need, s);
+    hipLaunchKernelGGL(need_blocks_kernel, dim3((n_keep + 255) / 256), dim3(256), 0, s, keep, n_keep, T, rows_per_blk, nblk, need);
 }
 
 __global__ void fill_f32_kernel(float* p, int64_t n, float v) {
diff --git a/proteingym_amd/csrc/model.h b/proteingym_amd/csrc/model.h
--- a/proteingym_amd/csrc/model.h
+++ b/proteingym_amd/csrc/model.h
@@ -28,6 +28,13 @@
     float *c_ln_w = nullptr, *c_ln_b = nullptr, *c_bqkv = nullptr, *c_bo = nullptr;
     W16 c_wqkv16, c_wo16;
     float *q_ln = nullptr, *k_ln = nullptr;
+};
+
+struct Layer0Share {
+    int G = 0;
+    const int32_t* seq_group = nullptr;
+    const int32_t* mask_rel = nullptr;
+    const int32_t* src_rows = nullptr;
 };
 
 struct ProfEvent {
@@ -84,7 +91,9 @@
     size_t qk16_plane = 0, vt16_plane = 0;
     int32_t* nonfinite = nullptr;
     int gemm_variant = 0;
-    int keep_rows = 1;
+    int keep_rows = 2;
+    unsigned char* att_need = nullptr;
+    int share_layer0 = 1;
     int last_B = 0, last_T = 0;
     int dh = kHeadDim;
     int rot_halves = 1;
@@ -115,6 +124,9 @@
     int64_t* mut_off = nullptr;
     float* table = nullptr;
     double* scores = nullptr;
+    std::vector<int> share_G;
+    std::vector<size_t> share_src_off;
+    int32_t *share_group = nullptr, *share_src = nullptr;
 };
 
 struct pgmi_pppl {
@@ -199,10 +211,11 @@
 int create_esm(pgmi_model* m, const pgmi_config* cfg, const float* w, int64_t n_weights);
 int ensure_rotary(pgmi_model* m, int T);
 int upload_rotate_half(pgmi_model* m, int n);
-int run_encoder(pgmi_model* m, int B, int T, const int32_t* keep = nullptr, int n_keep = 0, bool* compacted = nullptr);
+int run_encoder(pgmi_model* m, int B, int T, const int32_t* keep = nullptr, int n_keep = 0, bool* compacted = nullptr,
+                const Layer0Share* share = nullptr);
 int head_hidden(pgmi_model* m, int R, const int32_t* row_idx);
 int run_head(pgmi_model* m, int R, const int32_t* row_idx);
-int run_rows(pgmi_model* m, int B, int T, int R, const int32_t* row_idx);
+int run_rows(pgmi_model* m, int B, int T, int R, const int32_t* row_idx, const Layer0Share* share = nullptr);
 int create_tranception(pgmi_model* m, const pgmi_config* cfg, const float* w, int64_t n_weights);
 int create_progen2(pgmi_model* m, const pgmi_config* cfg, const float* w, int64_t n_weights, int rotary_dim);
 int create_gpt(pgmi_model* m, const pgmi_config* cfg, const float* w, int64_t n_weights, int pos_kind);
```
